# kurhula/pyABC

Measured on AMD Instinct MI355X. Metric: accepted particles/sec/generation, higher is better.
Workload: dtype f32 (f16x3-limb MFMA, f32-grade)

## Files before the change

### include/abcgpu.h

```cpp
#ifndef ABCGPU_H
#define ABCGPU_H

#include <stddef.h>
#include <stdint.h>

#ifdef __cplusplus
extern "C" {
#endif

#define ABC_OK 0
#define ABC_ERR_INVALID (-1)
#define ABC_ERR_HIP (-2)
#define ABC_ERR_WORKSPACE (-3)
#define ABC_ERR_NOT_ENOUGH_PARTICLES (-4)
#define ABC_ERR_UNSUPPORTED (-5)
#define ABC_ERR_COMM (-6)

#define ABC_MAX_D 2048

#define ABC_PREC_F64 0
#define ABC_PREC_F32 1
#define ABC_PREC_X3 2

#define ABC_PRIOR_FLAT (-1)
#define ABC_PRIOR_NORM 0
#define ABC_PRIOR_UNIFORM 1
#define ABC_PRIOR_EXPON 2
#define ABC_PRIOR_LAPLACE 3
#define ABC_PRIOR_LOGNORM 4
#define ABC_PRIOR_GAMMA 5
#define ABC_PRIOR_BETA 6
#define ABC_PRIOR_HOST 7

const char* abc_last_error(void);
int abc_version(void);

int abc_profile_begin(void);
int abc_profile_end(double* total_ms, int64_t* launches);
#define ABC_PROF_DENSITY 0
#define ABC_PROF_CANDIDATES 1
#define ABC_PROF_REGEN 2
#define ABC_PROF_RESCUE 3
int abc_profile_channel(int channel, double* total_ms, int64_t* launches);

size_t abc_weighted_moments_workspace(int64_t N, int d);
int abc_weighted_moments(const double* X, const double* w, int64_t N, int d,
                         double* out, void* ws, size_t ws_bytes, void* stream);

size_t abc_scan_workspace(int64_t N);
int abc_inclusive_scan_f64(const double* in, double* out, int64_t N, void* ws,
                           size_t ws_bytes, void* stream);

size_t abc_normalize_weights_workspace(int64_t N);
int abc_normalize_weights(double* w, int64_t N, double* stats, void* ws,
                          size_t ws_bytes, void* stream);

size_t abc_mvn_packed_bytes(int64_t N, int r, int prec);
int abc_mvn_pack_population(const double* X, const double* w, int64_t N, int d,
                            const double* mu, const double* U, int r,
                            double log_w_shift, const double* log_w_shift_dev,
                            int prec, void* packed, double* range, void* stream);
int abc_mvn_fit(const double* moments, int d, double scaling, int bw_rule,
                double* cov, double* evec, double* evals, double* U, double* L,
                double* stats, void* stream);
size_t abc_mvn_logpdf_workspace(int64_t M, int64_t N, int r, int prec);
int abc_mvn_x3_layout(int r, int* kslots, int* tiles_per_wave);
int abc_mvn_x3_max_exponent(void);
int abc_mvn_logpdf(const double* x, int64_t M, int d, const void* packed,
                   const double* X, const double* w, int64_t N,
                   const double* mu, const double* U, int r, int prec,
                   double log_const, double log_w_shift, double* out,
                   const int64_t* hint_rows, void* ws, size_t ws_bytes,
                   void* stream);
int abc_mvn_logpdf_direct(const double* x, int64_t M, const double* X,
                          const double* w, int64_t N, int d, const double* U,
                          int r, const double* V, int nv, double support_tol,
                          double log_const, double* out, void* stream);

int abc_cdf_guide(const double* cdf, int64_t N, int32_t* guide, void* stream);
int abc_propose(const double* X, const double* cdf, const int32_t* guide,
                int64_t N, int d, const double* L, const int32_t* prior_kind,
                const double* prior_params, uint64_t seed, uint32_t generation,
                int64_t idx0, int64_t B, int max_attempts, double* theta,
                double* prior_logpdf, int64_t* ancestor, int32_t* attempts,
                void* stream);
int abc_prior_logpdf(const double* theta, int64_t B, int d,
                     const int32_t* prior_kind, const double* prior_params,
                     double* out, void* stream);
int abc_prior_uniforms(const int32_t* attempts, double* u, int64_t B, int k,
                       uint64_t seed, uint32_t generation, int64_t idx0,
                       void* stream);

int abc_simulate_linear_gaussian(const double* theta, int64_t B, int d, int S,
                                 const int32_t* src, const double* a,
                                 const double* sigma, uint64_t seed,
                                 uint32_t generation, int64_t idx0, double* x,
                                 void* stream);

int abc_pnorm(const double* x, int64_t B, int S, const double* x0,
              const double* wf, double p, double* d, void* stream);

int abc_mask_gave_up(double* dist, const int32_t* attempts, int64_t B,
                     int max_attempts, double value, void* stream);

size_t abc_compact_workspace(int64_t B);
int abc_accept_compact(const double* d, int64_t B, double eps, int64_t* idx,
                       int64_t* count, void* ws, size_t ws_bytes,
                       void* stream);
typedef struct abc_candidate_spec {
  int d;
  int S;
  const double* X;
  const double* cdf;
  const int32_t* guide;
  int64_t N;
  const double* L;
  int per_particle_L;
  const int32_t* prior_kind;
  const double* prior_params;
  int max_attempts;
  const int32_t* src;
  const double* a;
  const double* sigma;
  const double* x0;
  const double* wf;
  double p;
  uint64_t seed;
  uint32_t generation;
  const void* anc_table;
  const double* support_box;
} abc_candidate_spec;
int abc_prior_support_box(const int32_t* prior_kind, const double* prior_params, int d,
                          double* box, void* stream);
int64_t abc_ancestor_table_bytes(int64_t N, int d);
int abc_ancestor_table(const double* X, const double* cdf, int64_t N, int d,
                       void* table, size_t table_bytes, void* stream);
size_t abc_candidates_workspace(int64_t B);
int abc_candidates_round(const abc_candidate_spec* spec, int64_t idx0,
                         int64_t B, double eps, const double* eps_dev,
                         double eps_scale, int filter, int64_t cap,
                         int64_t* idx, int64_t* count, double* rec_x,
                         void* ws, size_t ws_bytes, void* stream);
int abc_round_keep(const int64_t* counts, int nranks, int rank, int64_t need, int64_t* keep,
                   void* stream);
int abc_candidates_regen(const abc_candidate_spec* spec, int64_t idx0,
                         const int64_t* idx, int64_t n, const int64_t* n_dev,
                         double* theta, double* prior_logpdf, int64_t* ancestor,
                         double* x, double* dist, void* stream);

size_t abc_candidates_propose_workspace(void);
int abc_candidates_propose(const abc_candidate_spec* spec, int64_t idx0, int64_t B,
                           double* theta, double* prior_logpdf, int64_t* ancestor,
                           int32_t* attempts, void* ws, size_t ws_bytes, void* stream);

int abc_pnorm_accept(const double* x, int64_t B, int S, const double* x0,
                     const double* wf, double p, double eps, const int32_t* attempts,
                     int max_attempts, int64_t cap, int64_t* idx, int64_t* count,
                     void* ws, size_t ws_bytes, void* stream);

#define ABC_AGG_MAX_TERMS 16
int abc_aggregate_distance(const double* x, int64_t B, int S, const double* x0,
                           const double* wf, const double* p, const double* c, int K,
                           double* d, double* terms, void* stream);
int abc_aggregate_accept(const double* x, int64_t B, int S, const double* x0,
                         const double* wf, const double* p, const double* c, int K,
                         double eps, const int32_t* attempts, int max_attempts, int64_t cap,
                         int64_t* idx, int64_t* count, void* ws, size_t ws_bytes,
                         void* stream);

int abc_gather_rows(const double* in, const int64_t* idx, int64_t n, int cols,
                    double* out, void* stream);
int abc_gather_rows_batch(int n_arrays, const double* const* ins,
                          const int* cols, double* const* outs,
                          const int64_t* out_row0, const int64_t* idx,
                          int64_t n, void* stream);

int abc_importance_weights(const double* prior_logpdf,
                           const double* trans_logpdf,
                           const double* acc_weights, int64_t A, double scale,
                           double* w, void* stream);

size_t abc_sort_pairs_workspace(int64_t N);
int abc_sort_pairs_f64(const double* keys, const double* vals, int64_t N,
                       double* keys_out, double* vals_out, void* ws,
                       size_t ws_bytes, void* stream);
size_t abc_weighted_quantile_workspace(int64_t N);
int abc_weighted_quantile(const double* points, const double* w, int64_t N,
                          double alpha, double* q, void* ws, size_t ws_bytes,
                          void* stream);
size_t abc_weighted_quantile_sorted_workspace(int64_t N);
int abc_weighted_quantile_sorted(const double* points, const double* w, int64_t N,
                                 double alpha, double* q, void* ws, size_t ws_bytes,
                                 void* stream);

size_t abc_column_stats_workspace(int64_t R, int S);
int abc_column_std(const double* X, int64_t R, int S, double* out, void* ws,
                   size_t ws_bytes, void* stream);
int abc_column_mad(const double* X, int64_t R, int S, double* out, void* ws,
                   size_t ws_bytes, void* stream);

enum { ABC_SCALE_MAD, ABC_SCALE_MEAN_AD, ABC_SCALE_STD, ABC_SCALE_BIAS, ABC_SCALE_RMSD,
       ABC_SCALE_MAD_TO_OBS, ABC_SCALE_MEAN_AD_TO_OBS, ABC_SCALE_CMAD,
       ABC_SCALE_CMEAN_AD, ABC_SCALE_STD_TO_OBS };
size_t abc_column_scale_workspace(int kind, int64_t R, int S);
int abc_column_scale(int kind, const double* X, int64_t R, int S, const double* x0,
                     double* out, void* ws, size_t ws_bytes, void* stream);

int abc_column_span(const double* V, int64_t R, int K, double* out, void* ws,
                    size_t ws_bytes, void* stream);

size_t abc_local_fit_workspace(int64_t N, int d);
int abc_local_fit(const double* X, const double* w, int64_t N, int d,
                  int64_t k, double scaling, double eps, double* covs,
                  double* inv_covs, double* dets, double* chol,
                  double* log_norm, void* ws, size_t ws_bytes, void* stream);
#define ABC_FIT_KNN 1
#define ABC_FIT_LIST 2
#define ABC_FIT_DENSE 4
#define ABC_FIT_DEFER 8
#define ABC_FIT_DENSE_REJECTED 16
#define ABC_FIT_SELECT_FALLBACK 32
int abc_local_fit_route(void);
size_t abc_local_logpdf_workspace(int64_t M, int64_t N, int d);
int abc_local_logpdf(const double* x, int64_t M, const double* X,
                     const double* w, int64_t N, int d, const double* inv_covs,
                     const double* log_norm, double* out, void* ws,
                     size_t ws_bytes, void* stream);
int abc_local_logpdf_route(int64_t M, int64_t N, int d, void* ws, size_t ws_bytes,
                           void* stream, int64_t* direct, double* bound);
int abc_local_propose(const double* X, const double* cdf,
                      const int32_t* guide, int64_t N, int d,
                      const double* chol, const int32_t* prior_kind,
                      const double* prior_params, uint64_t seed,
                      uint32_t generation, int64_t idx0, int64_t B,
                      int max_attempts, double* theta, double* prior_logpdf,
                      int64_t* ancestor, int32_t* attempts, void* stream);

size_t abc_bootstrap_cv_workspace(int64_t N);
int abc_bootstrap_cv(const double* logdens, int64_t B, int64_t N,
                     const double* w, double scale, double* variation,
                     double* cv, void* ws, size_t ws_bytes, void* stream);

int abc_kernel_logpdf(const double* x, int64_t B, int S, const int32_t* cols,
                      int K, const double* x0k, int kind, const double* par,
                      const double* U, int r, double c, int ret_lin,
                      double* out, void* stream);
int abc_stochastic_accept(const double* dens, int64_t B, double pdf_norm,
                          double temperature, int scale_log, int apply_iw,
                          uint64_t seed, uint32_t generation, int64_t idx0,
                          double* key, double* accw, void* stream);
size_t abc_temper_workspace(void);
int abc_temper_sums(const double* dens, const double* lr,
                    const double* lr_sub, int64_t R, double pdf_norm, int scale_log, int mode, double beta,
                    double shift, double* out, void* ws, size_t ws_bytes,
                    void* stream);

#define ABC_COMM_ID_BYTES 128
#define ABC_COMM_F64 0
#define ABC_COMM_I64 1
#define ABC_COMM_SUM 0
#define ABC_COMM_MAX 1
#define ABC_COMM_MIN 2
int abc_comm_unique_id(void* id);
int abc_comm_init(void** comm, int nranks, int rank, const void* id);
int abc_comm_destroy(void* comm);
int abc_comm_allgather(void* comm, const void* send, void* recv, size_t bytes,
                       void* stream);
int abc_comm_allreduce(void* comm, const void* send, void* recv, size_t count,
                       int dtype, int op, void* stream);
int abc_comm_broadcast(void* comm, void* buf, size_t bytes, int root, void* stream);

#ifdef __cplusplus
}
#endif
#endif
```

### pyabc_amd/_native.py

```python
import ctypes as C
import os
import threading

_HERE = os.path.dirname(os.path.abspath(__file__))
LIB_PATH = os.environ.get("ABCGPU_LIB", os.path.join(_HERE, "libabcgpu.so"))

P = C.c_void_p
I64 = C.c_int64
I32 = C.c_int
D = C.c_double
U64 = C.c_uint64
U32 = C.c_uint32
SZ = C.c_size_t

SIGNATURES = {
    "abc_last_error": (C.c_char_p, []),
    "abc_version": (I32, []),
    "abc_profile_begin": (I32, []),
    "abc_profile_end": (I32, [P, P]),
    "abc_profile_channel": (I32, [I32, P, P]),
    "abc_weighted_moments_workspace": (SZ, [I64, I32]),
    "abc_weighted_moments": (I32, [P, P, I64, I32, P, P, SZ, P]),
    "abc_scan_workspace": (SZ, [I64]),
    "abc_inclusive_scan_f64": (I32, [P, P, I64, P, SZ, P]),
    "abc_normalize_weights_workspace": (SZ, [I64]),
    "abc_normalize_weights": (I32, [P, I64, P, P, SZ, P]),
    "abc_mvn_packed_bytes": (SZ, [I64, I32, I32]),
    "abc_mvn_x3_layout": (I32, [I32, P, P]),
    "abc_mvn_x3_max_exponent": (I32, []),
    "abc_mvn_pack_population": (I32, [P, P, I64, I32, P, P, I32, D, P, I32, P, P,
                                      P]),
    "abc_mvn_fit": (I32, [P, I32, D, I32, P, P, P, P, P, P, P]),
    "abc_mvn_logpdf_workspace": (SZ, [I64, I64, I32, I32]),
    "abc_mvn_logpdf": (I32, [P, I64, I32, P, P, P, I64, P, P, I32, I32, D, D,
                             P, P, P, SZ, P]),
    "abc_mvn_logpdf_direct": (I32, [P, I64, P, P, I64, I32, P, I32, P, I32,
                                    D, D, P, P]),
    "abc_cdf_guide": (I32, [P, I64, P, P]),
    "abc_ancestor_table_bytes": (I64, [I64, I32]),
    "abc_ancestor_table": (I32, [P, P, I64, I32, P, SZ, P]),
    "abc_propose": (I32, [P, P, P, I64, I32, P, P, P, U64, U32, I64, I64, I32,
                          P, P, P, P, P]),
    "abc_prior_logpdf": (I32, [P, I64, I32, P, P, P, P]),
    "abc_prior_uniforms": (I32, [P, P, I64, I32, U64, U32, I64, P]),
    "abc_simulate_linear_gaussian": (I32, [P, I64, I32, I32, P, P, P, U64,
                                           U32, I64, P, P]),
    "abc_pnorm": (I32, [P, I64, I32, P, P, D, P, P]),
    "abc_mask_gave_up": (I32, [P, P, I64, I32, D, P]),
    "abc_compact_workspace": (SZ, [I64]),
    "abc_accept_compact": (I32, [P, I64, D, P, P, P, SZ, P]),
    "abc_candidates_workspace": (SZ, [I64]),
    "abc_prior_support_box": (I32, [P, P, I32, P, P]),
    "abc_round_keep": (I32, [P, I32, I32, I64, P, P]),
    "abc_candidates_round": (I32, [P, I64, I64, D, P, D, I32, I64, P, P, P, P, SZ, P]),
    "abc_candidates_regen": (I32, [P, I64, P, I64, P, P, P, P, P, P, P]),
    "abc_pnorm_accept": (I32, [P, I64, I32, P, P, D, D, P, I32, I64, P, P, P, SZ, P]),
    "abc_aggregate_distance": (I32, [P, I64, I32, P, P, P, P, I32, P, P, P]),
    "abc_aggregate_accept": (I32, [P, I64, I32, P, P, P, P, I32, D, P, I32, I64, P, P, P,
                                   SZ, P]),
    "abc_column_span": (I32, [P, I64, I32, P, P, SZ, P]),
    "abc_candidates_propose_workspace": (SZ, []),
    "abc_candidates_propose": (I32, [P, I64, I64, P, P, P, P, P, SZ, P]),
    "abc_gather_rows": (I32, [P, P, I64, I32, P, P]),
    "abc_gather_rows_batch": (I32, [I32, P, P, P, P, P, I64, P]),
    "abc_importance_weights": (I32, [P, P, P, I64, D, P, P]),
    "abc_sort_pairs_workspace": (SZ, [I64]),
    "abc_sort_pairs_f64": (I32, [P, P, I64, P, P, P, SZ, P]),
    "abc_weighted_quantile_workspace": (SZ, [I64]),
    "abc_weighted_quantile": (I32, [P, P, I64, D, P, P, SZ, P]),
    "abc_weighted_quantile_sorted_workspace": (SZ, [I64]),
    "abc_weighted_quantile_sorted": (I32, [P, P, I64, D, P, P, SZ, P]),
    "abc_column_stats_workspace": (SZ, [I64, I32]),
    "abc_column_std": (I32, [P, I64, I32, P, P, SZ, P]),
    "abc_column_mad": (I32, [P, I64, I32, P, P, SZ, P]),
    "abc_column_scale_workspace": (SZ, [I32, I64, I32]),
    "abc_column_scale": (I32, [I32, P, I64, I32, P, P, P, SZ, P]),
    "abc_local_fit_workspace": (SZ, [I64, I32]),
    "abc_local_fit": (I32, [P, P, I64, I32, I64, D, D, P, P, P, P, P, P, SZ,
                            P]),
    "abc_local_fit_route": (I32, []),
    "abc_local_logpdf_workspace": (SZ, [I64, I64, I32]),
    "abc_local_logpdf": (I32, [P, I64, P, P, I64, I32, P, P, P, P, SZ, P]),
    "abc_local_logpdf_route": (I32, [I64, I64, I32, P, SZ, P, P, P]),
    "abc_local_propose": (I32, [P, P, P, I64, I32, P, P, P, U64, U32, I64,
                                I64, I32, P, P, P, P, P]),
    "abc_bootstrap_cv_workspace": (SZ, [I64]),
    "abc_bootstrap_cv": (I32, [P, I64, I64, P, D, P, P, P, SZ, P]),
    "abc_kernel_logpdf": (I32, [P, I64, I32, P, I32, P, I32, P, P, I32, D,
                                I32, P, P]),
    "abc_stochastic_accept": (I32, [P, I64, D, D, I32, I32, U64, U32, I64,
                                    P, P, P]),
    "abc_temper_workspace": (SZ, []),
    "abc_temper_sums": (I32, [P, P, P, I64, D, I32, I32, D, D, P, P, SZ, P]),
    "abc_comm_unique_id": (I32, [P]),
    "abc_comm_init": (I32, [P, I32, I32, P]),
    "abc_comm_destroy": (I32, [P]),
    "abc_comm_allgather": (I32, [P, P, P, SZ, P]),
    "abc_comm_allreduce": (I32, [P, P, P, SZ, I32, I32, P]),
    "abc_comm_broadcast": (I32, [P, P, SZ, I32, P]),
}



class CandidateSpec(C.Structure):
    _fields_ = [("d", C.c_int), ("S", C.c_int),
                ("X", P), ("cdf", P), ("guide", P), ("N", I64),
                ("L", P), ("per_particle_L", C.c_int),
                ("prior_kind", P), ("prior_params", P), ("max_attempts", C.c_int),
                ("src", P), ("a", P), ("sigma", P),
                ("x0", P), ("wf", P), ("p", D),
                ("seed", U64), ("generation", U32), ("anc_table", P),
                ("support_box", P)]


ABC_OK = 0
ABC_ERR_INVALID = -1
ABC_ERR_HIP = -2
ABC_ERR_WORKSPACE = -3
ABC_ERR_NOT_ENOUGH_PARTICLES = -4
ABC_ERR_UNSUPPORTED = -5
ABC_ERR_COMM = -6
ABC_AGG_MAX_TERMS = 16
ABC_COMM_ID_BYTES = 128
ABC_COMM_F64, ABC_COMM_I64 = 0, 1
ABC_COMM_SUM, ABC_COMM_MAX, ABC_COMM_MIN = 0, 1, 2
ABC_PROF_DENSITY, ABC_PROF_CANDIDATES, ABC_PROF_REGEN, ABC_PROF_RESCUE = 0, 1, 2, 3
(ABC_FIT_KNN, ABC_FIT_LIST, ABC_FIT_DENSE, ABC_FIT_DEFER, ABC_FIT_DENSE_REJECTED,
 ABC_FIT_SELECT_FALLBACK) = 1, 2, 4, 8, 16, 32
ABC_PREC_F64 = 0
ABC_PREC_F32 = 1
ABC_PREC_X3 = 2
(ABC_SCALE_MAD, ABC_SCALE_MEAN_AD, ABC_SCALE_STD, ABC_SCALE_BIAS, ABC_SCALE_RMSD,
 ABC_SCALE_MAD_TO_OBS, ABC_SCALE_MEAN_AD_TO_OBS, ABC_SCALE_CMAD, ABC_SCALE_CMEAN_AD,
 ABC_SCALE_STD_TO_OBS) = range(10)
SCALE_KINDS = {"mad": ABC_SCALE_MAD, "mean_ad": ABC_SCALE_MEAN_AD,
               "std": ABC_SCALE_STD, "bias": ABC_SCALE_BIAS,
               "rmsd": ABC_SCALE_RMSD, "mad_to_obs": ABC_SCALE_MAD_TO_OBS,
               "mean_ad_to_obs": ABC_SCALE_MEAN_AD_TO_OBS,
               "cmad": ABC_SCALE_CMAD, "cmean_ad": ABC_SCALE_CMEAN_AD,
               "std_to_obs": ABC_SCALE_STD_TO_OBS}

PRIOR_KINDS = {"norm": 0, "uniform": 1, "expon": 2, "laplace": 3,
               "lognorm": 4, "gamma": 5, "beta": 6, "host": 7}


class NativeError(RuntimeError):
    def __init__(self, fn, code, msg):
        super().__init__(f"{fn} failed ({code}): {msg}")
        self.code = code


_lib = None
_lock = threading.Lock()


def load():
    global _lib
    if _lib is not None:
        return _lib
    with _lock:
        if _lib is not None:
            return _lib
        if not os.path.exists(LIB_PATH):
            raise ImportError(
                f"libabcgpu.so not found at {LIB_PATH}; build it with "
                "`python -m pyabc_amd.build` (hipcc, gfx950)")
        lib = C.CDLL(LIB_PATH)
        for name, (res, args) in SIGNATURES.items():
            fn = getattr(lib, name)
            fn.restype = res
            fn.argtypes = args
        _lib = lib
    return _lib


def call(name, *args):
    lib = load()
    rc = getattr(lib, name)(*args)
    if rc != ABC_OK:
        msg = lib.abc_last_error().decode(errors="replace")
        if rc == ABC_ERR_INVALID:
            raise ValueError(f"{name}: {msg}")
        raise NativeError(name, rc, msg)
    return rc


def query(name, *args):
    return int(getattr(load(), name)(*args))
```

### pyabc_amd/csrc/abc_candidate.h

```cpp
#pragma once
#include "abc_common.h"

#pragma clang fp contract(off)

namespace abc {

constexpr double LOG_SQRT_2PI = 0.91893853320467274178;
constexpr uint32_t SLOTS_PER_ATTEMPT = 65536;
constexpr uint32_t SLOT_ANCESTOR = 0;
constexpr uint32_t SLOT_PERTURB = 1;
constexpr uint32_t SLOT_PRIOR = 32;
constexpr uint32_t SLOT_SIM = 0x40000000u;

__device__ __forceinline__ void normals4(uint64_t g, uint32_t slot, uint32_t gen,
                                         uint64_t seed, double n[4], int need = 4,
                                         const float* tab = BM_TAB) {
  u32x4 r = philox(g, slot, gen, seed);
  box_muller(r.x, r.y, n[0], n[1], tab);
  if (need > 2) box_muller(r.z, r.w, n[2], n[3], tab);
}

__device__ __forceinline__ void perturb_words(int p, const u32x4& anc, u32x4& r, uint64_t g,
                                              uint32_t s0, uint32_t gen, uint64_t seed,
                                              uint32_t& wa, uint32_t& wb) {
  if (p == 0) {
    wa = anc.z;
    wb = anc.w;
    return;
  }
  const int p1 = p - 1;
  if ((p1 & 1) == 0) r = philox(g, s0 + SLOT_PERTURB + (uint32_t)(p1 >> 1), gen, seed);
  wa = (p1 & 1) ? r.z : r.x;
  wb = (p1 & 1) ? r.w : r.y;
}

__device__ __noinline__ double prior_logpdf1(int kind, const double* p, double x) {
  switch (kind) {
    case ABC_PRIOR_FLAT:
      return 0.0;
    case ABC_PRIOR_NORM: {
      double y = (x - p[0]) / p[1];
      return -0.5 * (y * y) - LOG_SQRT_2PI - log(p[1]);
    }
    case ABC_PRIOR_UNIFORM: {
      double y = (x - p[0]) / p[1];
      return (y >= 0.0 && y <= 1.0) ? -log(p[1]) : -INFINITY;
    }
    case ABC_PRIOR_EXPON: {
      double y = (x - p[0]) / p[1];
      return (y >= 0.0) ? -y - log(p[1]) : -INFINITY;
    }
    case ABC_PRIOR_LAPLACE: {
      double y = (x - p[0]) / p[1];
      return -fabs(y) - log(2.0 * p[1]);
    }
    case ABC_PRIOR_LOGNORM: {
      double y = (x - p[1]) / p[2];
      if (!(y > 0.0)) return -INFINITY;
      const double lg = log(y), ly = lg / p[0];
      return -0.5 * ly * ly - lg - log(p[0]) - LOG_SQRT_2PI - log(p[2]);
    }
    case ABC_PRIOR_GAMMA: {
      double a = p[0], y = (x - p[1]) / p[2];
      if (y < 0.0) return -INFINITY;
      if (y == 0.0) return a < 1.0 ? INFINITY : (a == 1.0 ? -log(p[2]) : -INFINITY);
      const double t1 = (a == 1.0) ? 0.0 : (a - 1.0) * log(y);
      return t1 - y - lgamma(a) - log(p[2]);
    }
    case ABC_PRIOR_BETA: {
      double a = p[0], b = p[1], y = (x - p[2]) / p[3];
      if (y < 0.0 || y > 1.0) return -INFINITY;
      double lb = lgamma(a) + lgamma(b) - lgamma(a + b);
      double t1 = (a == 1.0) ? 0.0 : (a - 1.0) * log(y);
      double t2 = (b == 1.0) ? 0.0 : (b - 1.0) * log1p(-y);
      return t1 + t2 - lb - log(p[3]);
    }
    case ABC_PRIOR_HOST:
      return (x >= p[0] && x <= p[1]) ? 0.0 : -INFINITY;
  }
  return NAN;
}

__device__ __forceinline__ bool prior_in_support1(int kind, const double* p, double x) {
  switch (kind) {
    case ABC_PRIOR_FLAT:
      return true;
    case ABC_PRIOR_NORM: {
      double y = (x - p[0]) / p[1];
      return y * y < INFINITY;
    }
    case ABC_PRIOR_UNIFORM: {
      double y = (x - p[0]) / p[1];
      return y >= 0.0 && y <= 1.0;
    }
    case ABC_PRIOR_EXPON: {
      double y = (x - p[0]) / p[1];
      return y >= 0.0 && y < INFINITY;
    }
    case ABC_PRIOR_LAPLACE: {
      double y = (x - p[0]) / p[1];
      return fabs(y) < INFINITY;
    }
    case ABC_PRIOR_LOGNORM: {
      double y = (x - p[1]) / p[2];
      return y > 0.0 && y < INFINITY;
    }
    case ABC_PRIOR_GAMMA: {
      double y = (x - p[1]) / p[2];
      return (y > 0.0 && y < INFINITY) || (y == 0.0 && p[0] <= 1.0);
    }
    case ABC_PRIOR_BETA: {
      double y = (x - p[2]) / p[3];
      if (!(y >= 0.0 && y <= 1.0)) return false;
      if (y == 0.0 && p[0] > 1.0) return false;
      if (y == 1.0 && p[1] > 1.0) return false;
      return true;
    }
    case ABC_PRIOR_HOST:
      return x >= p[0] && x <= p[1];
  }
  return false;
}

__device__ inline double gamma_draw(double a, uint64_t g, uint32_t base, uint32_t gen,
                                    uint64_t seed) {
  double boost = 1.0;
  uint32_t it = 0;
  if (a < 1.0) {
    u32x4 r = philox(g, base + 500, gen, seed);
    boost = pow(uniform01(r.x), 1.0 / a);
    a += 1.0;
  }
  const double dd = a - 1.0 / 3.0, c = 1.0 / sqrt(9.0 * dd);
  for (; it < 480; ++it) {
    u32x4 r = philox(g, base + it, gen, seed);
    double n0, n1;
    box_muller(r.x, r.y, n0, n1);
    double v = 1.0 + c * n0;
    if (v <= 0.0) continue;
    v = v * v * v;
    double u = uniform01(r.z);
    if (log(u) < 0.5 * n0 * n0 + dd - dd * v + dd * log(v)) return dd * v * boost;
  }
  return dd * boost;
}

__device__ __noinline__ double prior_draw1(int kind, const double* p, uint64_t g,
                                     uint32_t base, uint32_t gen, uint64_t seed) {
  u32x4 r = philox(g, base, gen, seed);
  double n0, n1;
  switch (kind) {
    case ABC_PRIOR_NORM:
      box_muller(r.x, r.y, n0, n1);
      return p[0] + p[1] * n0;
    case ABC_PRIOR_UNIFORM:
      return p[0] + p[1] * uniform53(r.x, r.y);
    case ABC_PRIOR_EXPON:
      return p[0] - p[1] * log(uniform01(r.x));
    case ABC_PRIOR_LAPLACE: {
      double u = uniform01(r.x) - 0.5;
      return p[0] - p[1] * copysign(1.0, u) * log1p(-2.0 * fabs(u));
    }
    case ABC_PRIOR_LOGNORM:
      box_muller(r.x, r.y, n0, n1);
      return p[1] + p[2] * exp(p[0] * n0);
    case ABC_PRIOR_GAMMA:
      return p[1] + p[2] * gamma_draw(p[0], g, base + 1, gen, seed);
    case ABC_PRIOR_BETA: {
      double x = gamma_draw(p[0], g, base + 1, gen, seed);
      double y = gamma_draw(p[1], g, base + 1 + 256, gen, seed);
      return p[2] + p[3] * x / (x + y);
    }
    case ABC_PRIOR_HOST:
      return p[2];
  }
  return NAN;
}

__device__ __forceinline__ double prior_logpdf(const int32_t* kind,
                                               const double* params, int d,
                                               const double* th) {
  double s = 0.0;
  for (int k = 0; k < d; ++k) s += prior_logpdf1(kind[k], params + 4 * k, th[k]);
  return s;
}

__device__ __forceinline__ int64_t upper_bound(const double* cdf, int64_t N,
                                               double target) {
  int64_t lo = 0, hi = N;
  while (lo < hi) {
    int64_t mid = (lo + hi) >> 1;
    if (cdf[mid] > target) hi = mid; else lo = mid + 1;
  }
  return lo < N ? lo : N - 1;
}

__device__ __forceinline__ int64_t ancestor_search(const double* __restrict__ cdf,
                                                   const int32_t* __restrict__ guide,
                                                   int64_t N, double total,
                                                   double target) {
  if (guide == nullptr) return upper_bound(cdf, N, target);
  const double step = total / (double)N;
  int64_t k = (int64_t)floor(target / step) - 1;
  k = k < 0 ? 0 : (k > N - 1 ? N - 1 : k);
  int64_t lo = guide[k];
  int64_t hi = k + 3 < N ? (int64_t)guide[k + 3] + 1 : N;
  while (lo < hi) {
    const int64_t mid = (lo + hi) >> 1;
    if (cdf[mid] > target) hi = mid; else lo = mid + 1;
  }
  return lo < N ? lo : N - 1;
}

struct AncestorBracket { int64_t lo, hi; };
__device__ __forceinline__ AncestorBracket ancestor_bracket(const int32_t* __restrict__ guide,
                                                            int64_t N, double total,
                                                            double target) {
  if (guide == nullptr) return {0, N};
  const double step = total / (double)N;
  int64_t k = (int64_t)floor(target / step) - 1;
  k = k < 0 ? 0 : (k > N - 1 ? N - 1 : k);
  const int64_t k3 = k + 3 < N ? k + 3 : N - 1;
  const int64_t lo = guide[k];
  const int64_t g3 = guide[k3];
  return {lo, k + 3 < N ? g3 + 1 : N};
}
__device__ __forceinline__ int64_t ancestor_finish(const double* __restrict__ cdf, int64_t N,
                                                   double target, AncestorBracket b) {
  int64_t lo = b.lo, hi = b.hi;
  while (lo < hi) {
    const int64_t mid = (lo + hi) >> 1;
    if (cdf[mid] > target) hi = mid; else lo = mid + 1;
  }
  return lo < N ? lo : N - 1;
}

__device__ __forceinline__ int64_t table_finish(const double* __restrict__ rec, int rs, int d,
                                                int64_t N, double target, AncestorBracket b) {
  int64_t lo = b.lo, hi = b.hi;
  while (lo < hi) {
    const int64_t mid = (lo + hi) >> 1;
    if (rec[mid * rs + d] > target) hi = mid; else lo = mid + 1;
  }
  return lo < N ? lo : N - 1;
}

__device__ __forceinline__ uint64_t dkey(double x) {
  const uint64_t u = (uint64_t)__double_as_longlong(x);
  return (u >> 63) ? ~u : (u | (1ull << 63));
}
__device__ __forceinline__ double dval(uint64_t k) {
  const uint64_t u = (k >> 63) ? (k & ~(1ull << 63)) : ~k;
  return __longlong_as_double((long long)u);
}
__device__ __forceinline__ void support_bounds_wave(int kind, const double* pg, double* lo_hi) {
  const int lane = threadIdx.x & 63;
  double p[4];
#pragma unroll
  for (int i = 0; i < 4; ++i) p[i] = pg[i];
  double c;
  switch (kind) {
    case ABC_PRIOR_UNIFORM: c = p[0] + 0.5 * p[1]; break;
    case ABC_PRIOR_EXPON: c = p[0] + p[1]; break;
    case ABC_PRIOR_LOGNORM: case ABC_PRIOR_GAMMA: c = p[1] + p[2]; break;
    case ABC_PRIOR_BETA: c = p[2] + 0.5 * p[3]; break;
    case ABC_PRIOR_NORM: case ABC_PRIOR_LAPLACE: c = p[0]; break;
    case ABC_PRIOR_HOST: c = p[2]; break;
    default: c = 0.0;
  }
  auto pos = [](double v) { return v > 0.0 && v < INFINITY; };
  bool dom = true;
  switch (kind) {
    case ABC_PRIOR_NORM: case ABC_PRIOR_UNIFORM: case ABC_PRIOR_EXPON: case ABC_PRIOR_LAPLACE:
      dom = pos(p[1]); break;
    case ABC_PRIOR_LOGNORM: case ABC_PRIOR_GAMMA: dom = pos(p[0]) && pos(p[2]); break;
    case ABC_PRIOR_BETA: dom = pos(p[0]) && pos(p[1]) && pos(p[3]); break;
    default: break;
  }
  if (!dom || !prior_in_support1(kind, p, c)) {
    bool found = false;
    if (dom && fabs(c) < INFINITY) {
      const uint64_t kc0 = dkey(c);
#pragma unroll
      for (int s = 0; s < 2; ++s) {
        double c2 = dval(s ? kc0 - 1 : kc0 + 1);
        if (c2 == c) c2 = dval(s ? kc0 - 2 : kc0 + 2);
        if (!found && prior_in_support1(kind, p, c2)) {
          c = c2;
          found = true;
        }
      }
    }
    if (!found) {
      if (lane == 0) { lo_hi[0] = INFINITY; lo_hi[1] = -INFINITY; }
      return;
    }
  }
  auto turn = [&](uint64_t lo, uint64_t hi, bool up) {
    while (hi - lo > 1) {
      const uint64_t span = hi - lo;
      const uint64_t step = span / 65 > 0 ? span / 65 : 1;
      const uint64_t m = lo + step * (uint64_t)(lane + 1);
      const bool inside = m < hi;
      const bool pr = inside ? (prior_in_support1(kind, p, dval(m)) == up) : true;
      const unsigned long long bal = __ballot(pr);
      if (bal == 0ull) {
        lo = lo + step * 64ull;
        continue;
      }
      const int f = __ffsll((long long)bal) - 1;
      const uint64_t mf = lo + step * (uint64_t)(f + 1);
      const uint64_t new_hi = mf < hi ? mf : hi;
      const uint64_t new_lo = f == 0 ? lo : lo + step * (uint64_t)f;
      lo = new_lo;
      hi = new_hi;
    }
    return hi;
  };
  const uint64_t kc = dkey(c);
  uint64_t lo_key;
  if (prior_in_support1(kind, p, -INFINITY)) lo_key = dkey(-INFINITY);
  else lo_key = turn(dkey(-INFINITY), kc, true);
  uint64_t hi_key;
  if (prior_in_support1(kind, p, INFINITY)) hi_key = dkey(INFINITY);
  else hi_key = turn(kc, dkey(INFINITY), false) - 1;
  if (lane == 0) { lo_hi[0] = dval(lo_key); lo_hi[1] = dval(hi_key); }
}

struct ProposalArgs {
  const double* X;
  const double* cdf;
  const int32_t* guide;
  int64_t N;
  const double* L;
  const int32_t* kind;
  const double* params;
  int d;
  int max_attempts;
  uint64_t seed;
  uint32_t gen;
  const double* rec = nullptr;
  const int32_t* bguide = nullptr;
  int rs = 0;
  int64_t G = 0;
  const double* xmax = nullptr;
};

constexpr int ANC_HDR = 256;
__host__ __device__ inline int anc_rs(int d) { return (d + 1 + 15) / 16 * 16; }
__host__ __device__ inline int64_t anc_bins(int64_t N) {
  const int64_t g = 4 * N;
  return g < (int64_t)0x7FFFFFF0 ? g : (int64_t)0x7FFFFFF0;
}
__device__ __forceinline__ int64_t anc_bin(double x, double inv_step, int64_t G) {
  const double b = x * inv_step;
  return b >= (double)G ? G : (int64_t)b;
}

constexpr int PROP_MVN = 0, PROP_LOCAL = 1, PROP_PRIOR = 2;
using PropModes = std::integer_sequence<int, PROP_MVN, PROP_LOCAL, PROP_PRIOR>;
inline int proposal_mode(const double* X, bool per_particle_L) {
  return X == nullptr ? PROP_PRIOR : (per_particle_L ? PROP_LOCAL : PROP_MVN);
}

using CandDims = std::integer_sequence<int, 1, 2, 3, 4, 5, 6, 8, 10, 12, 16>;

template <class F>
void dispatch_candidate(int d, int mode, F&& f) {
  auto with_d = [&](auto D) { dispatch_int(PropModes{}, mode, [&](auto MODE) { f(D, MODE); }); };
  if (!dispatch_int(CandDims{}, d, with_d)) with_d(std::integral_constant<int, 0>{});
}

struct SimDistArgs {
  const int32_t* src;
  const double* a;
  const double* sigma;
  const double* x0;
  const double* wf;
  double p;
  int S;
};

constexpr int SIM_SMAX = 256;
constexpr int LT_DMAX = 16;
struct BlockConsts {
  float bmt[BM_TAB_SIZE];
  double LT[LT_DMAX * LT_DMAX];
  double box[2 * 64];
  double2 as[SIM_SMAX];
  double2 wx[SIM_SMAX];
  int32_t src[SIM_SMAX];
  double total;
  double inv_step;
  int lazy;
};

template <int D, int MODE, bool BOX_FROM_SRC = false>
__device__ __forceinline__ void stage_block_consts(BlockConsts& C, const ProposalArgs& A,
                                                   const SimDistArgs* M,
                                                   const double* box_src) {
  const int t = threadIdx.x, nt = blockDim.x;
  const int d = D > 0 ? D : A.d;
  for (int k = t; k < BM_TAB_SIZE; k += nt) C.bmt[k] = BM_TAB[k];
  if (MODE == PROP_MVN && D > 0 && D <= LT_DMAX)
    for (int e = t; e < d * d; e += nt) C.LT[(e % d) * d + e / d] = A.L[e];
  if (BOX_FROM_SRC) {
    for (int k = t; k < 2 * d; k += nt) C.box[k] = box_src[k];
  } else {
    for (int k = t >> 6; k < d; k += nt >> 6)
      support_bounds_wave(A.kind[k], A.params + 4 * k, C.box + 2 * k);
  }
  if (M)
    for (int k = t; k < M->S && k < SIM_SMAX; k += nt) {
      C.as[k] = make_double2(M->a[k], M->sigma[k]);
      C.wx[k] = make_double2(M->wf[k], M->x0[k]);
      C.src[k] = M->src[k];
    }
  if (t == 0) {
    const double total = (MODE != PROP_PRIOR) ? A.cdf[A.N - 1] : 0.0;
    C.total = total;
    C.inv_step = (MODE != PROP_PRIOR && A.rec) ? (double)A.G / total : 0.0;
  }
  __syncthreads();
}

template <int D, int MODE, bool TABLE = false>
__device__ __forceinline__ int propose_one(const ProposalArgs& A, const BlockConsts& C,
                                           uint64_t g, double* th, int64_t& j) {
  constexpr bool LT_LDS = MODE == PROP_MVN && D > 0 && D <= LT_DMAX;
  const int d = D > 0 ? D : A.d;
  j = -1;
  const double total = C.total;
  for (int att = 0; att < A.max_attempts; ++att) {
    const uint32_t s0 = (uint32_t)att * SLOTS_PER_ATTEMPT;
    int oz = 0;
    asm volatile("" : "+s"(oz));
    const double* LT = C.LT + oz;
    const double* box = C.box + oz;
    if (MODE == PROP_PRIOR) {
#pragma unroll
      for (int k = 0; k < (D > 0 ? D : d); ++k)
        th[k] = prior_draw1(A.kind[k], A.params + 4 * k, g,
                            s0 + SLOT_PRIOR + 512u * k, A.gen, A.seed);
    } else {
      const u32x4 ra = philox(g, s0 + SLOT_ANCESTOR, A.gen, A.seed);
      u32x4 r = ra;
      const double target = uniform53(ra.x, ra.y) * total;
      AncestorBracket br;
      if (TABLE) {
        const int64_t kt = anc_bin(target, C.inv_step, A.G);
        br = {A.bguide[kt], A.bguide[kt + 1]};
      } else {
        br = ancestor_bracket(A.guide, A.N, total, target);
      }
#pragma unroll
      for (int k = 0; k < (D > 0 ? D : d); ++k) th[k] = 0.0;
      const double* Lj = A.L;
      if (MODE == PROP_LOCAL) {
        j = TABLE ? table_finish(A.rec, A.rs, d, A.N, target, br)
                  : ancestor_finish(A.cdf, A.N, target, br);
        Lj = A.L + j * d * d;
      }
      auto pair = [&](int q) {
        uint32_t wa, wb;
        perturb_words(q >> 1, ra, r, g, s0, A.gen, A.seed, wa, wb);
        double n0, n1;
        box_muller(wa, wb, n0, n1, C.bmt);
        const bool two = q + 1 < d;
#pragma unroll
        for (int k = 0; k < (D > 0 ? D : d); ++k) {
          if (k >= q) {
            const double l0 = LT_LDS ? LT[q * d + k] : Lj[k * d + q];
            th[k] = fma(l0, n0, th[k]);
          }
          if (two && k >= q + 1) {
            const double l1 = LT_LDS ? LT[(q + 1) * d + k] : Lj[k * d + q + 1];
            th[k] = fma(l1, n1, th[k]);
          }
        }
      };
#pragma unroll 1
      for (int q = 0; q < d; q += 2) pair(q);
      if (MODE != PROP_LOCAL)
        j = TABLE ? table_finish(A.rec, A.rs, d, A.N, target, br)
                  : ancestor_finish(A.cdf, A.N, target, br);
      const double* Xj = TABLE ? A.rec + j * A.rs : A.X + j * d;
#pragma unroll
      for (int k = 0; k < (D > 0 ? D : d); ++k) th[k] = Xj[k] + th[k];
    }
    bool ok = true;
#pragma unroll
    for (int k = 0; k < (D > 0 ? D : d); ++k)
      ok = ok & (box[2 * k] <= th[k]) & (th[k] <= box[2 * k + 1]);
    if (ok) return att + 1;
  }
  return A.max_attempts + 1;
}

constexpr int LAZY_KT = 4;

template <int D, int MODE>
__device__ __forceinline__ bool lazy_filter_ok(const BlockConsts& C, const ProposalArgs& A,
                                               const SimDistArgs& M) {
  if constexpr (MODE != PROP_MVN || D <= LAZY_KT || D > LT_DMAX) {
    return false;
  } else {
    if (A.xmax == nullptr || M.S <= 4) return false;
    bool ok = true;
    for (int k = 0; k < 4; ++k) ok = ok && C.src[k] >= 0 && C.src[k] < LAZY_KT;
    const double xm = *A.xmax;
    for (int k = LAZY_KT; k < D; ++k) {
      double ls = 0.0;
      for (int q = 0; q <= k; ++q) ls += fabs(C.LT[q * D + k]);
      const double b = (xm + 7.6 * ls) * 1.000001 + 1e-300;
      ok = ok && (C.box[2 * k] <= -b) && (b <= C.box[2 * k + 1]);
    }
    return ok;
  }
}

__device__ __forceinline__ double pterm(double v, double p) {
#pragma clang fp contract(off)
  return (p == 1.0) ? v : (p == 2.0 ? v * v : pow(v, p));
}
template <int PK = 0>
__device__ __forceinline__ double pnorm_acc(double s, double v, double p) {
#pragma clang fp contract(off)
  if constexpr (PK == 2) return s + v * v;
  return isinf(p) ? fmax(s, v) : s + pterm(v, p);
}
template <int PK = 0>
__device__ __forceinline__ double pnorm_finish(double s, double p) {
#pragma clang fp contract(off)
  if constexpr (PK == 2) return sqrt(s);
  return isinf(p) ? s : ((p == 1.0) ? s : (p == 2.0 ? sqrt(s) : pow(s, 1.0 / p)));
}
__device__ __forceinline__ double pnorm_row(const double* xr, int S, const double* x0,
                                            const double* wf, double p) {
#pragma clang fp contract(off)
  double s = 0.0;
  if (isinf(p)) {
    for (int k = 0; k < S; ++k) s = fmax(s, fabs(wf[k] * (xr[k] - x0[k])));
    return pnorm_finish<0>(s, p);
  }
  for (int k = 0; k < S; ++k) s += pterm(fabs(wf[k] * (xr[k] - x0[k])), p);
  return pnorm_finish<0>(s, p);
}
constexpr int PNORM_ROWS = 8;
template <class F>
__device__ __forceinline__ void pnorm_wave_rows(const double* x, int64_t b0, int64_t B, int S,
                                                const double* x0, const double* wf, double p,
                                                F&& emit) {
#pragma clang fp contract(off)
  const int lane = threadIdx.x & 63;
  const bool inf = isinf(p);
  double s[PNORM_ROWS];
#pragma unroll
  for (int r = 0; r < PNORM_ROWS; ++r) s[r] = 0.0;
  for (int k = lane; k < S; k += 64) {
    const double wk = wf[k], ck = x0[k];
    double v[PNORM_ROWS];
#pragma unroll
    for (int r = 0; r < PNORM_ROWS; ++r) v[r] = b0 + r < B ? x[(b0 + r) * S + k] : ck;
#pragma unroll
    for (int r = 0; r < PNORM_ROWS; ++r) {
      const double a = fabs(wk * (v[r] - ck));
      s[r] = inf ? fmax(s[r], a) : s[r] + pterm(a, p);
    }
  }
#pragma unroll
  for (int r = 0; r < PNORM_ROWS; ++r) {
    const double t = inf ? wave_max(s[r]) : wave_sum(s[r]);
    if (lane == 0 && b0 + r < B) emit(r, pnorm_finish<0>(t, p));
  }
}

__device__ __forceinline__ double lg_stat(double a, double sigma, double th_src, double e) {
  return a * th_src + sigma * e;
}

template <int PK = 0>
__device__ __forceinline__ double sim_pnorm_range(const SimDistArgs& M, const BlockConsts& C,
                                                  const double* tsrc, int tstride,
                                                  uint64_t g, uint32_t gen,
                                                  uint64_t seed, int q0, int q1,
                                                  double s, double* x, int xoff = 0) {
  u32x4 r;
  if (q0 < q1 && (q0 & 3)) r = philox(g, SLOT_SIM + (uint32_t)(q0 >> 2), gen, seed);
#pragma unroll 1
  for (int q = q0; q < q1; q += 2) {
    if ((q & 3) == 0) r = philox(g, SLOT_SIM + (uint32_t)(q >> 2), gen, seed);
    double n2[2];
    box_muller((q & 2) ? r.z : r.x, (q & 2) ? r.w : r.y, n2[0], n2[1], C.bmt);
#pragma unroll
    for (int t = 0; t < 2; ++t) {
      const int k = q + t;
      if (k < q1) {
        const double2 as = C.as[k], wx = C.wx[k];
        const double xv = lg_stat(as.x, as.y, tsrc[C.src[k] * tstride], n2[t]);
        if (x) x[k - xoff] = xv;
        s = pnorm_acc<PK>(s, fabs(wx.x * (xv - wx.y)), M.p);
      }
    }
  }
  return s;
}

template <int D, int PK = 0>
__device__ __forceinline__ double sim_pnorm_regs(const SimDistArgs& M, const BlockConsts& C,
                                                 const double (&th)[D], uint64_t g,
                                                 uint32_t gen, uint64_t seed, int q0, int q1,
                                                 double s, double* x, int xoff = 0) {
  u32x4 r;
  if (q0 < q1 && (q0 & 3)) r = philox(g, SLOT_SIM + (uint32_t)(q0 >> 2), gen, seed);
#pragma unroll 1
  for (int q = q0; q < q1; q += 2) {
    if ((q & 3) == 0) r = philox(g, SLOT_SIM + (uint32_t)(q >> 2), gen, seed);
    double n2[2];
    box_muller((q & 2) ? r.z : r.x, (q & 2) ? r.w : r.y, n2[0], n2[1], C.bmt);
#pragma unroll
    for (int t = 0; t < 2; ++t) {
      const int k = q + t;
      if (k < q1) {
        const double2 as = C.as[k], wx = C.wx[k];
        const int sk = __builtin_amdgcn_readfirstlane(C.src[k]);
        const double xv = lg_stat(as.x, as.y, th[sk], n2[t]);
        if (x) x[k - xoff] = xv;
        s = pnorm_acc<PK>(s, fabs(wx.x * (xv - wx.y)), M.p);
      }
    }
  }
  return s;
}

template <int D, int PK = 0>
__device__ __forceinline__ double sim_pnorm(const SimDistArgs& M, const BlockConsts& C,
                                            const double* th, uint64_t g, uint32_t gen,
                                            uint64_t seed, int q0, int q1, double s, double* x,
                                            int xoff = 0) {
  if constexpr (D > 0) {
    return sim_pnorm_regs<D, PK>(M, C, *reinterpret_cast<const double(*)[D]>(th), g, gen, seed,
                                 q0, q1, s, x, xoff);
  } else {
    return sim_pnorm_range<PK>(M, C, th, 1, g, gen, seed, q0, q1, s, x, xoff);
  }
}

template <int D, int PK, int CG>
__device__ __forceinline__ void lazy_head_group(const ProposalArgs& A, const SimDistArgs& M,
                                                const BlockConsts& C, const uint64_t (&g)[CG],
                                                double eps, bool (&keep)[CG]) {
  constexpr int KT = LAZY_KT;
  static_assert(D > KT, "lazy_head_group: D > LAZY_KT");
  int oz = 0;
  asm volatile("" : "+s"(oz));
  const double* LT = C.LT + oz;
  const double* box = C.box + oz;
  double target[CG];
  int32_t glo[CG], ghi[CG];
  uint32_t az[CG], aw[CG];
#pragma unroll
  for (int c = 0; c < CG; ++c) {
    const u32x4 r = philox(g[c], SLOT_ANCESTOR, A.gen, A.seed);
    target[c] = uniform53(r.x, r.y) * C.total;
    az[c] = r.z;
    aw[c] = r.w;
    const int64_t kt = anc_bin(target[c], C.inv_step, A.G);
    glo[c] = A.bguide[kt];
    ghi[c] = A.bguide[kt + 1];
  }
  double th[CG][KT];
#pragma unroll
  for (int c = 0; c < CG; ++c) {
#pragma unroll
    for (int k = 0; k < KT; ++k) th[c][k] = 0.0;
    const u32x4 r = philox(g[c], SLOT_PERTURB, A.gen, A.seed);
#pragma unroll
    for (int q = 0; q < KT; q += 2) {
      double n0, n1;
      box_muller(q == 0 ? az[c] : r.x, q == 0 ? aw[c] : r.y, n0, n1, C.bmt);
#pragma unroll
      for (int k = 0; k < KT; ++k) {
        if (k >= q) th[c][k] = fma(LT[q * D + k], n0, th[c][k]);
        if (k >= q + 1) th[c][k] = fma(LT[(q + 1) * D + k], n1, th[c][k]);
      }
    }
  }
  const double* xh[CG];
#pragma unroll
  for (int c = 0; c < CG; ++c) {
    const int64_t j = table_finish(A.rec, A.rs, D, A.N, target[c],
                                   AncestorBracket{(int64_t)glo[c], (int64_t)ghi[c]});
    xh[c] = A.rec + j * A.rs;
  }
  double xv4[CG][KT];
#pragma unroll
  for (int c = 0; c < CG; ++c)
#pragma unroll
    for (int k = 0; k < KT; ++k) xv4[c][k] = xh[c][k];
  double e[CG][4];
#pragma unroll
  for (int c = 0; c < CG; ++c) {
    const u32x4 r = philox(g[c], SLOT_SIM, A.gen, A.seed);
    box_muller(r.x, r.y, e[c][0], e[c][1], C.bmt);
    box_muller(r.z, r.w, e[c][2], e[c][3], C.bmt);
  }
#pragma unroll
  for (int c = 0; c < CG; ++c) {
    bool ok = true;
#pragma unroll
    for (int k = 0; k < KT; ++k) {
      th[c][k] = xv4[c][k] + th[c][k];
      ok = ok & (box[2 * k] <= th[c][k]) & (th[c][k] <= box[2 * k + 1]);
    }
    double s = 0.0;
#pragma unroll
    for (int k = 0; k < 4; ++k) {
      const double2 as = C.as[k], wx = C.wx[k];
      const int sk = __builtin_amdgcn_readfirstlane(C.src[k]);
      const double xv = lg_stat(as.x, as.y, th[c][sk], e[c][k]);
      s = pnorm_acc<PK>(s, fabs(wx.x * (xv - wx.y)), M.p);
    }
    keep[c] = !ok || !(pnorm_finish<PK>(s, M.p) > eps);
  }
}

}
```

### pyabc_amd/csrc/abc_fused.hip

```cpp
#include "abc_candidate.h"
#include "abc_aggregate.h"

namespace abc {
namespace {

constexpr int FR_T = 256;
constexpr int FR_CPT = 8;
constexpr int FR_TILE = FR_T * FR_CPT;
constexpr int FR_WORDS = FR_TILE / 64;
constexpr int FR_CG = 2;

struct RoundArgs {
  ProposalArgs P;
  SimDistArgs M;
  const double* box;
  const double* eps_dev;
  double eps_scale;
};

template <int D, int MODE, int PK>
__device__ __forceinline__ double evaluate_full(const RoundArgs& A, const BlockConsts& C,
                                                uint64_t g,
                                                double* th, int64_t& j, int& att, double* x) {
  att = propose_one<D, MODE, true>(A.P, C, g, th, j);
  const double s = sim_pnorm<D, PK>(A.M, C, th, g, A.P.gen, A.P.seed, 0, A.M.S, 0.0, x);
  const double dist = pnorm_finish<PK>(s, A.M.p);
  return att <= A.P.max_attempts ? dist : NAN;
}

constexpr int XCH = 16;
template <int D, int MODE, int PK>
__device__ __forceinline__ double evaluate_staged(const RoundArgs& A, const BlockConsts& C,
                                                  uint64_t g, bool valid, double* th,
                                                  int64_t& j, int& att, double* out,
                                                  int nvalid, double (*stage)[XCH + 1]) {
  const int t = threadIdx.x;
  const int S = A.M.S;
  att = valid ? propose_one<D, MODE, true>(A.P, C, g, th, j) : A.P.max_attempts + 1;
  double s = 0.0;
  for (int k0 = 0; k0 < S; k0 += XCH) {
    const int k1 = k0 + XCH < S ? k0 + XCH : S;
    if (valid) s = sim_pnorm<D, PK>(A.M, C, th, g, A.P.gen, A.P.seed, k0, k1, s, stage[t], k0);
    __syncthreads();
    const int w = k1 - k0;
    for (int e = t; e < FR_T * w; e += FR_T) {
      const int r = e / w, c = e - r * w;
      if (r < nvalid) out[(int64_t)r * S + k0 + c] = stage[r][c];
    }
    __syncthreads();
  }
  const double dist = pnorm_finish<PK>(s, A.M.p);
  return att <= A.P.max_attempts ? dist : NAN;
}

__device__ __forceinline__ void flush_accept_words(const uint32_t* tbits, int nwords,
                                                   int64_t tile0, int64_t B, uint64_t* bits) {
  const int lane = threadIdx.x & 63, wave = threadIdx.x >> 6;
  if (wave == 0 && lane < nwords) {
    const uint64_t w = (uint64_t)tbits[2 * lane] | ((uint64_t)tbits[2 * lane + 1] << 32);
    const int64_t word = tile0 / 64 + lane;
    if (word * 64 < B) bits[word] = w;
  }
}

struct TileLds {
  uint32_t* tbits;
  uint16_t* queue;
  int& qn;
};
template <int D, int MODE, bool FILTER, int PK>
__device__ __forceinline__ void tile_body(const RoundArgs& A, const BlockConsts& C, double eps,
                                          int64_t idx0, int64_t B, int64_t tile0, int cpt,
                                          uint64_t* __restrict__ bits,
                                          double* __restrict__ rec_x, TileLds T) {
  constexpr int DM = D > 0 ? D : 64;
  const int tid = threadIdx.x;
  const int tn = cpt * FR_T;
  if (tid < tn / 32) T.tbits[tid] = 0u;
  if (tid == 0) T.qn = 0;
  __syncthreads();
  double th[DM];
  int64_t j;
  int att;
  if (FILTER) {
    bool lazy_done = false;
    if constexpr (MODE == PROP_MVN && D > LAZY_KT && D <= LT_DMAX) {
      if (C.lazy) {
#pragma unroll 1
        for (int it = 0; it < cpt; it += FR_CG) {
          uint64_t gs[FR_CG];
          bool keep[FR_CG];
#pragma unroll
          for (int c = 0; c < FR_CG; ++c) gs[c] = (uint64_t)(idx0 + tile0 + (it + c) * FR_T + tid);
          lazy_head_group<D, PK, FR_CG>(A.P, A.M, C, gs, eps, keep);
#pragma unroll
          for (int c = 0; c < FR_CG; ++c) {
            const int loc = (it + c) * FR_T + tid;
            if (keep[c] && tile0 + loc < B) {
              const int pos = atomicAdd(&T.qn, 1);
              T.queue[pos] = (uint16_t)loc;
            }
          }
        }
        lazy_done = true;
      }
    }
#pragma unroll 1
    for (int it = 0; it < (lazy_done ? 0 : cpt); ++it) {
      const int loc = it * FR_T + tid;
      const int64_t b = tile0 + loc;
      if (b < B) {
        const uint64_t g = (uint64_t)(idx0 + b);
        att = propose_one<D, MODE, true>(A.P, C, g, th, j);
        const double s = sim_pnorm<D, PK>(A.M, C, th, g, A.P.gen, A.P.seed, 0, 4, 0.0, nullptr);
        if (att <= A.P.max_attempts && !(pnorm_finish<PK>(s, A.M.p) > eps)) {
          const int pos = atomicAdd(&T.qn, 1);
          T.queue[pos] = (uint16_t)loc;
        }
      }
    }
    __syncthreads();
  }
  const int n = FILTER ? T.qn : tn;
#pragma unroll 1
  for (int i = tid; i < n; i += FR_T) {
    const int loc = FILTER ? (int)T.queue[i] : i;
    const int64_t b = tile0 + loc;
    if (b < B) {
      double* xr = rec_x ? rec_x + b * A.M.S : nullptr;
      const double dist = evaluate_full<D, MODE, PK>(A, C, (uint64_t)(idx0 + b), th, j, att,
                                                  xr);
      if (dist <= eps) atomicOr(&T.tbits[loc >> 5], 1u << (loc & 31));
    }
  }
  __syncthreads();
  flush_accept_words(T.tbits, tn / 64, tile0, B, bits);
}

constexpr int FR_CPT_TAIL = 2;
constexpr int FR_TILE_TAIL = FR_T * FR_CPT_TAIL;

struct TilePlan {
  int64_t nbig, ntiles;
  unsigned int grid;
};
__host__ __device__ inline void tile_span(int64_t t, int64_t nbig, int64_t& tile0, int& cpt) {
  if (t < nbig) { tile0 = t * FR_TILE; cpt = FR_CPT; }
  else { tile0 = nbig * FR_TILE + (t - nbig) * FR_TILE_TAIL; cpt = FR_CPT_TAIL; }
}

template <int D, int MODE, bool FILTER, int PK>
__device__ __forceinline__ void round_body(RoundArgs A, int64_t idx0, int64_t B,
                                           double eps_host, uint64_t* __restrict__ bits,
                                           unsigned int* __restrict__ ticket,
                                           int64_t nbig, int64_t ntiles,
                                           double* __restrict__ rec_x) {
  const double eps = A.eps_dev ? (*A.eps_dev) * A.eps_scale : eps_host;
  __shared__ BlockConsts C;
  __shared__ uint32_t tbits[FR_TILE / 32];
  __shared__ uint16_t queue[FR_TILE];
  __shared__ int qn;
  __shared__ int64_t s_tile;
  const TileLds T{tbits, queue, qn};
  stage_block_consts<D, MODE, true>(C, A.P, &A.M, A.box);
  if (FILTER) {
    if (threadIdx.x == 0) C.lazy = lazy_filter_ok<D, MODE>(C, A.P, A.M) ? 1 : 0;
  }
  const unsigned int limit = (unsigned int)(ntiles + gridDim.x - 1);
#pragma unroll 1
  for (;;) {
    if (threadIdx.x == 0) s_tile = (int64_t)atomicInc(ticket, limit);
    __syncthreads();
    const int64_t t = s_tile;
    if (t >= ntiles) break;
    int64_t tile0;
    int cpt;
    tile_span(t, nbig, tile0, cpt);
    tile_body<D, MODE, FILTER, PK>(A, C, eps, idx0, B, tile0, cpt, bits, rec_x, T);
    __syncthreads();
  }
}

template <int D, int MODE, int PK>
__device__ __forceinline__ void round_plain_body(RoundArgs A, int64_t idx0, int64_t B,
                                                 double eps_host, uint64_t* __restrict__ bits,
                                                 unsigned int* __restrict__ ticket,
                                                 int64_t nbig, int64_t ntiles,
                                                 double* __restrict__ rec_x) {
  const double eps = A.eps_dev ? (*A.eps_dev) * A.eps_scale : eps_host;
  constexpr int DM = D > 0 ? D : 64;
  __shared__ BlockConsts C;
  __shared__ uint32_t tbits[FR_TILE / 32];
  __shared__ int64_t s_tile;
  stage_block_consts<D, MODE, true>(C, A.P, &A.M, A.box);
  const int tid = threadIdx.x, lane = tid & 63, wave = tid >> 6;
  const unsigned int limit = (unsigned int)(ntiles + gridDim.x - 1);
  int64_t tile0 = 0;
  int cpt = 0, it = 0;
  bool started = false;
#pragma unroll 1
  for (;;) {
    if (it == cpt) {
      __syncthreads();
      if (started && wave == 0 && lane < cpt * (FR_T / 64)) {
        const uint64_t w = (uint64_t)tbits[2 * lane] | ((uint64_t)tbits[2 * lane + 1] << 32);
        const int64_t word = tile0 / 64 + lane;
        if (word * 64 < B) bits[word] = w;
      }
      if (tid == 0) s_tile = (int64_t)atomicInc(ticket, limit);
      __syncthreads();
      const int64_t t = (int64_t)(((uint64_t)(uint32_t)__builtin_amdgcn_readfirstlane(
                                       (int)(s_tile >> 32)) << 32) |
                                  (uint32_t)__builtin_amdgcn_readfirstlane((int)s_tile));
      if (t >= ntiles) break;
      tile_span(t, nbig, tile0, cpt);
      if (tid < FR_TILE / 32) tbits[tid] = 0u;
      __syncthreads();
      it = 0;
      started = true;
    }
    const int loc = it * FR_T + tid;
    const int64_t b = tile0 + loc;
    if (b < B) {
      double th[DM];
      int64_t j;
      int att;
      double* xr = rec_x ? rec_x + b * A.M.S : nullptr;
      const double dist = evaluate_full<D, MODE, PK>(A, C, (uint64_t)(idx0 + b), th, j, att, xr);
      if (dist <= eps) atomicOr(&tbits[loc >> 5], 1u << (loc & 31));
    }
    ++it;
  }
}

__host__ __device__ constexpr int fr_min_waves(bool filter, int D, int MODE, int PK) {
  return (!filter && PK == 2 && D == 10 && MODE != PROP_PRIOR) ? 6 : 1;
}

#define ABC_ROUND_KERNEL(NAME, FILTER, PK)                                                \
  template <int D, int MODE>                                                              \
  __global__ __launch_bounds__(FR_T, fr_min_waves(FILTER, D, MODE, PK))                   \
  void NAME(RoundArgs A, int64_t idx0, int64_t B,                                         \
                                               double eps, uint64_t* bits,                \
                                               unsigned int* ticket, int64_t nbig,        \
                                               int64_t ntiles, double* rec_x) {           \
    if (FILTER)                                                                           \
      round_body<D, MODE, true, PK>(A, idx0, B, eps, bits, ticket, nbig, ntiles, nullptr);\
    else                                                                                  \
      round_plain_body<D, MODE, PK>(A, idx0, B, eps, bits, ticket, nbig, ntiles, rec_x);  \
  }
ABC_ROUND_KERNEL(fused_round_plain, false, 0)
ABC_ROUND_KERNEL(fused_round_plain_p2, false, 2)
ABC_ROUND_KERNEL(fused_round_filter, true, 0)
ABC_ROUND_KERNEL(fused_round_filter_p2, true, 2)
#undef ABC_ROUND_KERNEL

constexpr int RG_MAX = 2048;
constexpr int RG_T = 256;

__global__ __launch_bounds__(RG_T) void bits_range_sum_kernel(
    const uint64_t* __restrict__ bits, int64_t nwords, int64_t wpr,
    int64_t* __restrict__ rtot) {
  __shared__ int ws[RG_T / 64];
  const int64_t w0 = (int64_t)blockIdx.x * wpr;
  const int64_t w1 = w0 + wpr < nwords ? w0 + wpr : nwords;
  int c = 0;
  for (int64_t w = w0 + threadIdx.x; w < w1; w += RG_T) c += __popcll(bits[w]);
#pragma unroll
  for (int o = 32; o > 0; o >>= 1) c += __shfl_xor(c, o, 64);
  if ((threadIdx.x & 63) == 0) ws[threadIdx.x >> 6] = c;
  __syncthreads();
  if (threadIdx.x == 0) {
    int64_t tot = 0;
    for (int q = 0; q < RG_T / 64; ++q) tot += ws[q];
    rtot[blockIdx.x] = tot;
  }
}

constexpr int WB = 32;
__global__ __launch_bounds__(256) void bits_write_ranges(
    const uint64_t* __restrict__ bits, int64_t nwords, int64_t wpr, int nranges,
    const int64_t* __restrict__ rtot, int64_t cap, int64_t* __restrict__ idx,
    int64_t* __restrict__ count) {
  const int lane = threadIdx.x & 63;
  const int r = blockIdx.x * 4 + (threadIdx.x >> 6);
  if (r >= nranges) return;
  int64_t off = 0;
  for (int q = lane; q < r; q += 64) off += rtot[q];
#pragma unroll
  for (int o = 32; o > 0; o >>= 1) off += __shfl_xor(off, o, 64);
  const int64_t mine = rtot[r];
  if (r == nranges - 1 && lane == 0) *count = off + mine;
  if (off >= cap || mine == 0) return;
  const int64_t w0 = (int64_t)r * wpr;
  const int64_t w1 = w0 + wpr < nwords ? w0 + wpr : nwords;
  for (int64_t b0 = w0; b0 < w1 && off < cap; b0 += 64 * WB) {
    uint64_t w[WB];
#pragma unroll
    for (int q = 0; q < WB; ++q) {
      const int64_t wd = b0 + 64 * q + lane;
      w[q] = wd < w1 ? bits[wd] : 0ull;
    }
#pragma unroll
    for (int q = 0; q < WB; ++q) {
      if (b0 + 64 * q >= w1 || off >= cap) break;
      const int c = __popcll(w[q]);
      int incl = c;
#pragma unroll
      for (int o = 1; o < 64; o <<= 1) {
        const int u = __shfl_up(incl, o, 64);
        if (lane >= o) incl += u;
      }
      int64_t pos = off + (incl - c);
      uint64_t m = w[q];
      const int64_t wd = b0 + 64 * q + lane;
      while (m != 0ull && pos < cap) {
        idx[pos++] = wd * 64 + (__ffsll((long long)m) - 1);
        m &= m - 1;
      }
      off += __shfl(incl, 63, 64);
    }
  }
}

__global__ __launch_bounds__(64) void support_box_kernel(const int32_t* __restrict__ kind,
                                                         const double* __restrict__ params,
                                                         int d, double* __restrict__ box) {
  const int k = blockIdx.x;
  if (k < d) support_bounds_wave(kind[k], params + 4 * k, box + 2 * k);
}

struct Ranges { int64_t nwords, wpr; int n; };
inline Ranges make_ranges(int64_t B, int64_t most, int64_t least) {
  Ranges r;
  r.nwords = ceil_div(B, 64);
  if (most > RG_MAX) most = RG_MAX;
  int64_t n = ceil_div(r.nwords, least);
  n = n < most ? n : most;
  n = n < 1 ? 1 : n;
  r.wpr = ceil_div(r.nwords, n);
  r.n = (int)ceil_div(r.nwords, r.wpr);
  return r;
}

inline TilePlan plan_tiles(int64_t B, int resident) {
  TilePlan p;
  const int64_t tail = 2 * (int64_t)resident * FR_TILE_TAIL;
  p.nbig = B > tail ? (B - tail) / FR_TILE : 0;
  p.ntiles = p.nbig + ceil_div(B - p.nbig * FR_TILE, FR_TILE_TAIL);
  p.grid = (unsigned int)(p.ntiles < resident ? p.ntiles : resident);
  return p;
}

template <int D, int MODE>
void launch_round(bool filt, bool p2, const RoundArgs& A, int64_t idx0, int64_t B, double eps,
                  uint64_t* bits, unsigned int* ticket, double* rec_x, hipStream_t s) {
  auto k = filt ? (p2 ? fused_round_filter_p2<D, MODE> : fused_round_filter<D, MODE>)
                : (p2 ? fused_round_plain_p2<D, MODE> : fused_round_plain<D, MODE>);
  const TilePlan p = plan_tiles(B, resident_blocks(k, FR_T));
  hipLaunchKernelGGL(k, dim3(p.grid), dim3(FR_T), 0, s, A, idx0, B, eps, bits, ticket, p.nbig,
                     p.ntiles, rec_x);
}

template <int D, int MODE>
__global__ __launch_bounds__(256) void fused_regen_kernel(
    RoundArgs A, int64_t idx0, const int64_t* __restrict__ idx, int64_t n,
    const int64_t* __restrict__ n_dev, double* __restrict__ theta, double* __restrict__ lp,
    int64_t* __restrict__ anc, double* __restrict__ x, double* __restrict__ dist) {
  constexpr int DM = D > 0 ? D : 64;
  __shared__ BlockConsts C;
  __shared__ double stage[FR_T][XCH + 1];
  if (n_dev && *n_dev < n) n = *n_dev > 0 ? *n_dev : 0;
  if ((int64_t)blockIdx.x * FR_T >= n) return;
  stage_block_consts<D, MODE>(C, A.P, &A.M, nullptr);
  const int d = D > 0 ? D : A.P.d;
  const int64_t i0 = (int64_t)blockIdx.x * FR_T;
  const int64_t i = i0 + threadIdx.x;
  const bool valid = i < n;
  const int nvalid = n - i0 < FR_T ? (int)(n - i0) : FR_T;
  double th[DM];
  int64_t j = -1;
  int att;
  const double dd = evaluate_staged<D, MODE, 0>(A, C, valid ? (uint64_t)(idx0 + idx[i]) : 0ull,
                                                valid, th, j, att, x + i0 * A.M.S, nvalid, stage);
  if (!valid) return;
#pragma unroll
  for (int k = 0; k < (D > 0 ? D : d); ++k) theta[i * d + k] = th[k];
  lp[i] = att <= A.P.max_attempts ? prior_logpdf(A.P.kind, A.P.params, d, th) : -INFINITY;
  if (anc) anc[i] = j;
  dist[i] = dd;
}

__global__ void round_keep_kernel(const int64_t* __restrict__ counts, int rank, int64_t need,
                                  int64_t* __restrict__ keep) {
  if (threadIdx.x != 0) return;
  int64_t left = need > 0 ? need : 0, k = 0;
  for (int q = 0; q <= rank; ++q) {
    const int64_t c = counts[q] > 0 ? counts[q] : 0;
    const int64_t take = c < left ? c : left;
    if (q == rank) k = take;
    left -= take;
  }
  *keep = k;
}

constexpr int FP_CPT = 4;
template <int D, int MODE>
__global__ __launch_bounds__(256) void fused_propose_kernel(
    RoundArgs A, int64_t idx0, int64_t B, double* __restrict__ theta,
    double* __restrict__ lp, int64_t* __restrict__ anc, int32_t* __restrict__ att_out) {
  constexpr int DM = D > 0 ? D : 64;
  __shared__ BlockConsts C;
  stage_block_consts<D, MODE, true>(C, A.P, nullptr, A.box);
  const int d = D > 0 ? D : A.P.d;
  for (int c = 0; c < FP_CPT; ++c) {
    const int64_t i = ((int64_t)blockIdx.x * FP_CPT + c) * FR_T + threadIdx.x;
    if (i >= B) break;
    double th[DM];
    int64_t j = -1;
    const int att = propose_one<D, MODE, true>(A.P, C, (uint64_t)(idx0 + i), th, j);
    double* row = theta + i * d;
#pragma unroll
    for (int k = 0; k < DM; ++k)
      if (k < d) row[k] = th[k];
    if (lp) lp[i] = att <= A.P.max_attempts ? prior_logpdf(A.P.kind, A.P.params, d, th) : -INFINITY;
    if (anc) anc[i] = j;
    if (att_out) att_out[i] = att;
  }
}

__host__ __device__ constexpr int pa_chunk_rows(int S) {
  return (65536 / ((S + 1) * 8)) >= FR_T ? FR_T : ((65536 / ((S + 1) * 8)) & ~1);
}
template <bool WIDE>
__global__ __launch_bounds__(FR_T) void pnorm_accept_kernel(
    const double* __restrict__ x, int64_t B, int S, const double* __restrict__ x0,
    const double* __restrict__ wf, double p, double eps, const int32_t* __restrict__ att,
    int max_attempts, uint64_t* __restrict__ bits) {
  __shared__ uint32_t tbits[FR_TILE / 32];
  const int tid = threadIdx.x;
  const int64_t tile0 = (int64_t)blockIdx.x * FR_TILE;
  if (tid < FR_TILE / 32) tbits[tid] = 0u;
  __syncthreads();
  auto ok = [&](int64_t b) { return att == nullptr || att[b] <= max_attempts; };
  if (!WIDE) {
    extern __shared__ double pa_rows[];
    const int S1 = S + 1;
    const int RC = pa_chunk_rows(S);
    const int n16 = RC * S / 2;
    const int per = (n16 + FR_T - 1) / FR_T;
    double2 hold[16];
    auto fetch = [&](int it) {
      const int64_t e0 = (tile0 + (int64_t)it * RC) * S;
      const int64_t eend = B * S;
#pragma unroll
      for (int q = 0; q < 16; ++q) {
        if (q >= per) break;
        const int piece = q * FR_T + tid;
        const int64_t e = e0 + 2 * (int64_t)piece;
        if (piece < n16 && e + 1 < eend) {
          hold[q] = *reinterpret_cast<const double2*>(x + e);
        } else if (piece < n16 && e < eend) {
          hold[q] = double2{x[e], 0.0};
        }
      }
    };
    auto stash = [&]() {
#pragma unroll
      for (int q = 0; q < 16; ++q) {
        if (q >= per) break;
        const int piece = q * FR_T + tid;
        if (piece < n16) {
          const int e = 2 * piece;
          const int r0 = e / S, k0 = e - r0 * S;
          pa_rows[r0 * S1 + k0] = hold[q].x;
          const int r1 = (e + 1) / S, k1 = e + 1 - r1 * S;
          pa_rows[r1 * S1 + k1] = hold[q].y;
        }
      }
    };
    const int64_t rows = B - tile0 < FR_TILE ? B - tile0 : FR_TILE;
    const int nchunk = (int)((rows + RC - 1) / RC);
    fetch(0);
#pragma unroll 1
    for (int it = 0; it < nchunk; ++it) {
      __syncthreads();
      stash();
      __syncthreads();
      if (it + 1 < nchunk) fetch(it + 1);
      const int loc = it * RC + tid;
      const int64_t b = tile0 + loc;
      if (tid < RC && loc < FR_TILE && b < B) {
        const double dist = pnorm_row(pa_rows + tid * S1, S, x0, wf, p);
        if (dist <= eps && ok(b)) atomicOr(&tbits[loc >> 5], 1u << (loc & 31));
      }
    }
  } else {
#pragma unroll 1
    for (int r0 = (tid >> 6) * PNORM_ROWS; r0 < FR_TILE; r0 += 4 * PNORM_ROWS) {
      const int64_t b0 = tile0 + r0;
      if (b0 >= B) break;
      pnorm_wave_rows(x, b0, B, S, x0, wf, p, [&](int r, double dist) {
        const int loc = r0 + r;
        if (dist <= eps && ok(b0 + r)) atomicOr(&tbits[loc >> 5], 1u << (loc & 31));
      });
    }
  }
  __syncthreads();
  flush_accept_words(tbits, FR_WORDS, tile0, B, bits);
}

constexpr int AGG_TILE_ROW = FR_T, AGG_TILE_WAVE = 64;
template <bool WIDE, bool SIMPLE>
__global__ __launch_bounds__(FR_T) void aggregate_accept_kernel(
    const double* __restrict__ x, int64_t B, int S, const double* __restrict__ x0,
    const double* __restrict__ wf, const AggTerms T, double eps,
    const int32_t* __restrict__ att, int max_attempts, uint64_t* __restrict__ bits) {
  constexpr int TILE = WIDE ? AGG_TILE_WAVE : AGG_TILE_ROW;
  __shared__ uint32_t tbits[TILE / 32];
  const int tid = threadIdx.x;
  const int64_t tile0 = (int64_t)blockIdx.x * TILE;
  if (tid < TILE / 32) tbits[tid] = 0u;
  __syncthreads();
  auto ok = [&](int64_t b) { return att == nullptr || att[b] <= max_attempts; };
  if (!WIDE) {
    const int64_t b = tile0 + tid;
    if (b < B) {
      const double dist = agg_row(x + b * S, S, x0, wf, T, [](int, double) {});
      if (dist <= eps && ok(b)) atomicOr(&tbits[tid >> 5], 1u << (tid & 31));
    }
  } else {
#pragma unroll 1
    for (int r0 = (tid >> 6) * PNORM_ROWS; r0 < TILE; r0 += 4 * PNORM_ROWS) {
      const int64_t b0 = tile0 + r0;
      if (b0 >= B) break;
      agg_wave_rows<SIMPLE>(x, b0, B, S, x0, wf, T, [](int, int, double) {},
                            [&](int r, double dist) {
        const int loc = r0 + r;
        if (dist <= eps && ok(b0 + r)) atomicOr(&tbits[loc >> 5], 1u << (loc & 31));
      });
    }
  }
  __syncthreads();
  flush_accept_words(tbits, TILE / 64, tile0, B, bits);
}

int write_ranges(const uint64_t* bits, const Ranges& rg, const int64_t* rtot, int64_t cap,
                 int64_t* idx, int64_t* count, hipStream_t s) {
  hipLaunchKernelGGL(bits_write_ranges, dim3((unsigned)ceil_div(rg.n, 4)), dim3(256), 0, s,
                     bits, rg.nwords, rg.wpr, rg.n, rtot, cap, idx, count);
  ABC_LAUNCHED();
  return ABC_OK;
}

int compact_accept_bits(const uint64_t* bits, int64_t* rtot, int64_t B, int64_t cap,
                        int64_t* idx, int64_t* count, hipStream_t s) {
  const Ranges rg = make_ranges(B, RG_MAX, RG_T);
  hipLaunchKernelGGL(bits_range_sum_kernel, dim3((unsigned)rg.n), dim3(RG_T), 0, s, bits,
                     rg.nwords, rg.wpr, rtot);
  ABC_LAUNCHED();
  return write_ranges(bits, rg, rtot, cap, idx, count, s);
}

__global__ __launch_bounds__(256) void anc_records_kernel(const double* __restrict__ X,
                                                          const double* __restrict__ cdf,
                                                          int64_t N, int d, int rs,
                                                          double* __restrict__ rec) {
  const int64_t e = (int64_t)blockIdx.x * 256 + threadIdx.x;
  if (e >= N * rs) return;
  const int64_t i = e / rs;
  const int k = (int)(e - i * rs);
  rec[e] = k < d ? X[i * d + k] : (k == d ? cdf[i] : 0.0);
}

constexpr int XMAX_BLOCKS = 512;
__global__ __launch_bounds__(256) void anc_xmax_kernel(const double* __restrict__ X,
                                                       int64_t n,
                                                       unsigned long long* __restrict__ xmax_bits) {
  __shared__ unsigned long long wm[4];
  unsigned long long a = 0ull;
  for (int64_t e = (int64_t)blockIdx.x * 256 + threadIdx.x; e < n; e += (int64_t)gridDim.x * 256) {
    const unsigned long long b = (unsigned long long)__double_as_longlong(fabs(X[e]));
    a = b > a ? b : a;
  }
#pragma unroll
  for (int o = 32; o > 0; o >>= 1) {
    const unsigned long long b = __shfl_xor(a, o, 64);
    a = b > a ? b : a;
  }
  if ((threadIdx.x & 63) == 0) wm[threadIdx.x >> 6] = a;
  __syncthreads();
  if (threadIdx.x == 0) {
    unsigned long long m = 0ull;
    for (int w = 0; w < 4; ++w) m = wm[w] > m ? wm[w] : m;
    atomicMax(xmax_bits, m);
  }
}

__global__ __launch_bounds__(256) void anc_guide_kernel(const double* __restrict__ cdf,
                                                        int64_t N, int64_t G,
                                                        int32_t* __restrict__ guide) {
  const int64_t k = (int64_t)blockIdx.x * 256 + threadIdx.x;
  if (k > G + 1) return;
  const double inv_step = (double)G / cdf[N - 1];
  int64_t lo = 0, hi = N;
  while (lo < hi) {
    const int64_t mid = (lo + hi) >> 1;
    if (anc_bin(cdf[mid], inv_step, G) >= k) hi = mid; else lo = mid + 1;
  }
  guide[k] = (int32_t)lo;
}

struct AncTable { const double* rec; const int32_t* guide; int rs; int64_t G; const double* xmax; };
inline AncTable anc_table_view(const void* t, int64_t N, int d) {
  AncTable v;
  v.xmax = static_cast<const double*>(t);
  v.rs = anc_rs(d);
  v.G = anc_bins(N);
  v.rec = reinterpret_cast<const double*>(static_cast<const char*>(t) + ANC_HDR);
  v.guide = reinterpret_cast<const int32_t*>(v.rec + N * v.rs);
  return v;
}

RoundArgs round_args(const abc_candidate_spec* s, const double* box) {
  RoundArgs A;
  A.box = box;
  A.eps_dev = nullptr;
  A.eps_scale = 1.0;
  A.P = ProposalArgs{s->X, s->cdf, s->guide, s->N, s->L, s->prior_kind,
                     s->prior_params, s->d, s->max_attempts, s->seed, s->generation};
  if (s->X && s->anc_table) {
    const AncTable v = anc_table_view(s->anc_table, s->N, s->d);
    A.P.rec = v.rec;
    A.P.bguide = v.guide;
    A.P.rs = v.rs;
    A.P.G = v.G;
    A.P.xmax = v.xmax;
  }
  A.M = SimDistArgs{s->src, s->a, s->sigma, s->x0, s->wf, s->p, s->S};
  return A;
}

int check_spec(const abc_candidate_spec* s) {
  ABC_CHECK_ARG(s != nullptr, "candidates: null spec");
  ABC_CHECK_ARG(s->d >= 1 && s->d <= 64 && s->S >= 1, "candidates: bad d/S");
  if (s->S > SIM_SMAX)
    return set_error(ABC_ERR_UNSUPPORTED, "candidates: S > %d (use the staged kernels)",
                     SIM_SMAX);
  ABC_CHECK_ARG(s->max_attempts >= 1 && s->max_attempts < (1 << 15),
                "candidates: bad max_attempts");
  ABC_CHECK_ARG(s->prior_kind && s->prior_params && s->src && s->a && s->sigma && s->x0 &&
                s->wf, "candidates: null pointer");
  ABC_CHECK_ARG(s->X == nullptr || (s->cdf && s->L && s->N >= 1),
                "candidates: population needs cdf, L, N");
  ABC_CHECK_ARG(s->p >= 1.0, "candidates: p < 1");
  ABC_CHECK_ARG(s->X == nullptr || s->anc_table, "candidates: population needs anc_table");
  return ABC_OK;
}

template <class F>
void dispatch_spec(const abc_candidate_spec* spec, F&& f) {
  dispatch_candidate(spec->d, proposal_mode(spec->X, spec->per_particle_L != 0), f);
}

}
}

using namespace abc;

struct RoundWs {
  unsigned int* ticket; int64_t* rtot; double* box; uint64_t* bits;
  void carve(Carver& c, int64_t B) {
    ticket = c.take<unsigned int>(64);
    rtot = c.take<int64_t>(RG_MAX);
    box = c.take<double>(128);
    bits = c.take<uint64_t>((size_t)ceil_div(B > 0 ? B : 1, FR_TILE) * FR_WORDS);
  }
};

extern "C" size_t abc_candidates_workspace(int64_t B) { return measure<RoundWs>(B); }

extern "C" int64_t abc_ancestor_table_bytes(int64_t N, int d) {
  if (N < 1 || d < 1) return 0;
  return ANC_HDR + N * anc_rs(d) * (int64_t)sizeof(double) +
         (anc_bins(N) + 2) * (int64_t)sizeof(int32_t);
}

extern "C" int abc_ancestor_table(const double* X, const double* cdf, int64_t N, int d,
                                  void* table, size_t table_bytes, void* stream) {
  ABC_CHECK_ARG(N >= 1 && N < (1ll << 31) && d >= 1 && d <= 64,
                "ancestor_table: bad N/d");
  ABC_CHECK_ARG(X && cdf && table, "ancestor_table: null pointer");
  ABC_CHECK_ARG(((uintptr_t)table & 127) == 0, "ancestor_table: table not 128-B aligned");
  if ((int64_t)table_bytes < abc_ancestor_table_bytes(N, d))
    return set_error(ABC_ERR_WORKSPACE, "ancestor_table: buffer too small");
  const AncTable v = anc_table_view(table, N, d);
  hipStream_t s = as_stream(stream);
  ABC_HIP(hipMemsetAsync(table, 0, ANC_HDR, s));
  hipLaunchKernelGGL(anc_records_kernel, dim3((unsigned)ceil_div(N * v.rs, 256)), dim3(256), 0,
                     s, X, cdf, N, d, v.rs, const_cast<double*>(v.rec));
  ABC_LAUNCHED();
  const int64_t nx = N * (int64_t)d;
  const int64_t xb = ceil_div(nx, 256) < XMAX_BLOCKS ? ceil_div(nx, 256) : XMAX_BLOCKS;
  hipLaunchKernelGGL(anc_xmax_kernel, dim3((unsigned)xb), dim3(256), 0, s, X, nx,
                     static_cast<unsigned long long*>(table));
  ABC_LAUNCHED();
  hipLaunchKernelGGL(anc_guide_kernel, dim3((unsigned)ceil_div(v.G + 2, 256)), dim3(256), 0, s,
                     cdf, N, v.G, const_cast<int32_t*>(v.guide));
  ABC_LAUNCHED();
  return ABC_OK;
}

extern "C" int abc_candidates_round(const abc_candidate_spec* spec, int64_t idx0,
                                    int64_t B, double eps, const double* eps_dev,
                                    double eps_scale, int filter, int64_t cap,
                                    int64_t* idx, int64_t* count, double* rec_x,
                                    void* ws, size_t ws_bytes, void* stream) {
  const int rc = check_spec(spec);
  if (rc != ABC_OK) return rc;
  ABC_CHECK_ARG(B >= 0 && cap >= 0 && count, "candidates_round: bad B/cap/count");
  ABC_CHECK_ARG(B < (1ll << 40), "candidates_round: B too large");
  ABC_CHECK_ARG(cap == 0 || idx, "candidates_round: null idx");
  RoundWs w;
  ABC_CARVE(w, "candidates_round", B);
  hipStream_t s = as_stream(stream);
  if (B == 0) {
    ABC_HIP(hipMemsetAsync(count, 0, sizeof(int64_t), s));
    return ABC_OK;
  }
  const double p = spec->p;
  const int filt = (filter && rec_x == nullptr && spec->S > 4 &&
                    (p == 1.0 || p == 2.0 || p == INFINITY)) ? 1 : 0;
  const int64_t nt = ceil_div(B, FR_TILE);
  ABC_CHECK_ARG(nt < (1ll << 31), "candidates_round: too many tiles");
  const double* box = spec->support_box;
  if (!box) {
    hipLaunchKernelGGL(support_box_kernel, dim3((unsigned)spec->d), dim3(64), 0, s,
                       spec->prior_kind, spec->prior_params, spec->d, w.box);
    ABC_LAUNCHED();
    box = w.box;
  }
  RoundArgs A = round_args(spec, box);
  A.eps_dev = eps_dev;
  A.eps_scale = eps_scale;
  profile_start(s, ABC_PROF_CANDIDATES);
  dispatch_spec(spec, [&](auto D, auto MODE) {
    launch_round<D(), MODE()>(filt != 0, p == 2.0, A, idx0, B, eps, w.bits, w.ticket, rec_x, s);
  });
  profile_stop(s, ABC_PROF_CANDIDATES);
  ABC_LAUNCHED();
  return compact_accept_bits(w.bits, w.rtot, B, cap, idx, count, s);
}

extern "C" int abc_pnorm_accept(const double* x, int64_t B, int S, const double* x0,
                                const double* wf, double p, double eps,
                                const int32_t* attempts, int max_attempts, int64_t cap,
                                int64_t* idx, int64_t* count, void* ws, size_t ws_bytes,
                                void* stream) {
  ABC_CHECK_ARG(S >= 1 && B >= 0 && p >= 1.0 && cap >= 0, "pnorm_accept: bad S/B/p/cap");
  ABC_CHECK_ARG(B < (1ll << 40), "pnorm_accept: B too large");
  ABC_CHECK_ARG(count && (cap == 0 || idx), "pnorm_accept: null pointer");
  RoundWs w;
  ABC_CARVE(w, "pnorm_accept", B);
  hipStream_t s = as_stream(stream);
  if (B == 0) {
    ABC_HIP(hipMemsetAsync(count, 0, sizeof(int64_t), s));
    return ABC_OK;
  }
  ABC_CHECK_ARG(x && x0 && wf, "pnorm_accept: null pointer");
  const int64_t nt = ceil_div(B, FR_TILE);
  ABC_CHECK_ARG(nt < (1ll << 31), "pnorm_accept: too many tiles");
  uint64_t* bits = w.bits;
  if (S <= 32)
    hipLaunchKernelGGL(pnorm_accept_kernel<false>, dim3((unsigned)nt), dim3(FR_T),
                       (size_t)pa_chunk_rows(S) * (S + 1) * sizeof(double), s, x, B, S, x0, wf, p, eps,
                       attempts, max_attempts, bits);
  else
    hipLaunchKernelGGL(pnorm_accept_kernel<true>, dim3((unsigned)nt), dim3(FR_T), 0, s, x, B,
                       S, x0, wf, p, eps, attempts, max_attempts, bits);
  ABC_LAUNCHED();
  return compact_accept_bits(bits, w.rtot, B, cap, idx, count, s);
}

extern "C" int abc_aggregate_accept(const double* x, int64_t B, int S, const double* x0,
                                    const double* wf, const double* p, const double* c, int K,
                                    double eps, const int32_t* attempts, int max_attempts,
                                    int64_t cap, int64_t* idx, int64_t* count, void* ws,
                                    size_t ws_bytes, void* stream) {
  AggTerms T;
  const int rc = agg_check_terms("aggregate_accept", S, p, c, K, T);
  if (rc != ABC_OK) return rc;
  ABC_CHECK_ARG(B >= 0 && cap >= 0, "aggregate_accept: bad B/cap");
  ABC_CHECK_ARG(B < (1ll << 40), "aggregate_accept: B too large");
  ABC_CHECK_ARG(count && (cap == 0 || idx), "aggregate_accept: null pointer");
  RoundWs w;
  ABC_CARVE(w, "aggregate_accept", B);
  hipStream_t s = as_stream(stream);
  if (B == 0) {
    ABC_HIP(hipMemsetAsync(count, 0, sizeof(int64_t), s));
    return ABC_OK;
  }
  ABC_CHECK_ARG(x && x0 && wf, "aggregate_accept: null pointer");
  const int64_t nt = ceil_div(B, S <= 32 ? AGG_TILE_ROW : AGG_TILE_WAVE);
  ABC_CHECK_ARG(nt < (1ll << 31), "aggregate_accept: too many tiles");
  auto launch = [&](auto kernel) {
    hipLaunchKernelGGL(kernel, dim3((unsigned)nt), dim3(FR_T), 0, s, x, B, S, x0, wf, T, eps,
                       attempts, max_attempts, w.bits);
  };
  if (S <= 32) launch(aggregate_accept_kernel<false, false>);
  else if (agg_simple(T.p, K)) launch(aggregate_accept_kernel<true, true>);
  else launch(aggregate_accept_kernel<true, false>);
  ABC_LAUNCHED();
  return compact_accept_bits(w.bits, w.rtot, B, cap, idx, count, s);
}

extern "C" int abc_prior_support_box(const int32_t* prior_kind, const double* prior_params,
                                     int d, double* box, void* stream) {
  ABC_CHECK_ARG(d >= 1 && d <= 64, "prior_support_box: bad d");
  ABC_CHECK_ARG(prior_kind && prior_params && box, "prior_support_box: null pointer");
  hipLaunchKernelGGL(support_box_kernel, dim3((unsigned)d), dim3(64), 0, as_stream(stream),
                     prior_kind, prior_params, d, box);
  ABC_LAUNCHED();
  return ABC_OK;
}

extern "C" int abc_round_keep(const int64_t* counts, int nranks, int rank, int64_t need,
                              int64_t* keep, void* stream) {
  ABC_CHECK_ARG(counts && keep && nranks >= 1 && rank >= 0 && rank < nranks,
                "round_keep: bad arguments");
  hipLaunchKernelGGL(round_keep_kernel, dim3(1), dim3(64), 0, as_stream(stream), counts, rank,
                     need, keep);
  ABC_LAUNCHED();
  return ABC_OK;
}

struct ProposeWs {
  double* box;
  void carve(Carver& c) { box = c.take<double>(128); }
};

extern "C" size_t abc_candidates_propose_workspace() { return measure<ProposeWs>(); }

extern "C" int abc_candidates_propose(const abc_candidate_spec* spec, int64_t idx0, int64_t B,
                                      double* theta, double* prior_logpdf, int64_t* ancestor,
                                      int32_t* attempts, void* ws, size_t ws_bytes,
                                      void* stream) {
  const int rc = check_spec(spec);
  if (rc != ABC_OK) return rc;
  ABC_CHECK_ARG(B >= 0 && B < (1ll << 40), "candidates_propose: bad B");
  if (B == 0) return ABC_OK;
  ABC_CHECK_ARG(theta, "candidates_propose: null pointer");
  ProposeWs w;
  ABC_CARVE(w, "candidates_propose");
  hipStream_t s = as_stream(stream);
  double* box = w.box;
  if (spec->support_box) {
    box = const_cast<double*>(spec->support_box);
  } else {
    hipLaunchKernelGGL(support_box_kernel, dim3((unsigned)spec->d), dim3(64), 0, s,
                       spec->prior_kind, spec->prior_params, spec->d, box);
    ABC_LAUNCHED();
  }
  const RoundArgs A = round_args(spec, box);
  const int64_t nb = ceil_div(B, (int64_t)FR_T * FP_CPT);
  ABC_CHECK_ARG(nb < (1ll << 31), "candidates_propose: too many blocks");
  dispatch_spec(spec, [&](auto D, auto MODE) {
    hipLaunchKernelGGL((fused_propose_kernel<D(), MODE()>), dim3((unsigned)nb), dim3(256), 0, s,
                       A, idx0, B, theta, prior_logpdf, ancestor, attempts);
  });
  ABC_LAUNCHED();
  return ABC_OK;
}

extern "C" int abc_candidates_regen(const abc_candidate_spec* spec, int64_t idx0,
                                    const int64_t* idx, int64_t n, const int64_t* n_dev,
                                    double* theta, double* prior_logpdf, int64_t* ancestor,
                                    double* x, double* dist, void* stream) {
  const int rc = check_spec(spec);
  if (rc != ABC_OK) return rc;
  ABC_CHECK_ARG(n >= 0, "candidates_regen: n < 0");
  if (n == 0) return ABC_OK;
  ABC_CHECK_ARG(idx && theta && prior_logpdf && x && dist, "candidates_regen: null pointer");
  const RoundArgs A = round_args(spec, nullptr);
  hipStream_t s = as_stream(stream);
  profile_start(s, ABC_PROF_REGEN);
  dispatch_spec(spec, [&](auto D, auto MODE) {
    hipLaunchKernelGGL((fused_regen_kernel<D(), MODE()>), dim3((unsigned)ceil_div(n, 256)),
                       dim3(256), 0, s, A, idx0, idx, n, n_dev, theta, prior_logpdf, ancestor, x,
                       dist);
  });
  profile_stop(s, ABC_PROF_REGEN);
  ABC_LAUNCHED();
  return ABC_OK;
}
```

### pyabc_amd/gpu.py

```python
import math

import numpy as np

from . import _native as nat

try:
    import torch
except ImportError:
    torch = None

F64 = None if torch is None else torch.float64
I64 = None if torch is None else torch.int64


class NoDeviceError(RuntimeError):
    pass


_have_device = False


def require_device():
    global _have_device
    if not _have_device:
        if torch is None or not torch.cuda.is_available():
            raise NoDeviceError("pyabc_amd GPU path needs an MI355X (HIP device)")
        nat.load()
        _have_device = True
    return torch.device("cuda", torch.cuda.current_device())


def stream_ptr():
    return torch._C._cuda_getCurrentRawStream(torch.cuda.current_device())


def p(t):
    if t is None:
        return None
    assert t.is_contiguous(), "kernels take contiguous tensors"
    return t.data_ptr()


_ws = {}


def workspace(nbytes, slot="main"):
    dev = torch.cuda.current_device()
    key = (dev, slot)
    buf = _ws.get(key)
    nbytes = max(int(nbytes), 256)
    if buf is None or buf.numel() < nbytes:
        buf = torch.zeros(int(nbytes * 1.25) + 256, dtype=torch.uint8,
                          device=f"cuda:{dev}")
        _ws[key] = buf
    return buf


class HostFuture:

    _events = {}

    def __init__(self, t, _record=True):
        self._h = torch.empty(t.shape, dtype=t.dtype, pin_memory=True)
        self._h.copy_(t, non_blocking=True)
        self._dev = t.device.index if t.is_cuda else torch.cuda.current_device()
        self._pooled = _record
        self._ev = None
        if _record:
            pool = HostFuture._events.setdefault(self._dev, [])
            self._ev = pool.pop() if pool else torch.cuda.Event()
            self._ev.record(torch.cuda.current_stream(self._dev))
        self._v = None

    @classmethod
    def group(cls, ts):
        futs = [cls(t, _record=False) for t in ts]
        if futs:
            ev = torch.cuda.Event()
            ev.record(torch.cuda.current_stream(futs[-1]._dev))
            for f in futs:
                f._ev = ev
        return futs

    def get(self):
        if self._v is None:
            self._ev.synchronize()
            self._v = self._h.numpy().copy()
            pool = HostFuture._events.setdefault(self._dev, [])
            if self._pooled and len(pool) < 64:
                pool.append(self._ev)
            self._h = self._ev = None
        return self._v

    def __deepcopy__(self, memo):
        return self

    def __getstate__(self):
        return {"_v": self.get(), "_h": None, "_ev": None}


_flat = {}


def flat_prior(d, device):
    key = (int(d), str(device))
    if key not in _flat:
        _flat[key] = (as_dev(np.full(d, -1), dtype=torch.int32, device=device),
                      torch.zeros(4 * d, dtype=F64, device=device))
    return _flat[key]


def as_dev(a, dtype=None, device=None):
    dtype = dtype or F64
    device = device or require_device()
    if isinstance(a, torch.Tensor):
        return a.to(device=device, dtype=dtype).contiguous()
    return torch.as_tensor(np.ascontiguousarray(a), dtype=dtype,
                           device=device).contiguous()



def weighted_moments(X, w, with_max=False):
    N, d = X.shape
    out = torch.empty(3 + d + d * d, dtype=F64, device=X.device)
    nb = nat.query("abc_weighted_moments_workspace", N, d)
    ws = workspace(nb)
    nat.call("abc_weighted_moments", p(X), p(w), N, d, p(out), p(ws), ws.numel(),
             stream_ptr())
    o = out.cpu().numpy()
    res = (o[0], o[1], o[2:2 + d].copy(), o[2 + d:2 + d + d * d].reshape(d, d).copy())
    return res + (o[2 + d + d * d],) if with_max else res


def inclusive_scan(x, out=None):
    n = x.numel()
    out = torch.empty_like(x) if out is None else out
    nb = nat.query("abc_scan_workspace", n)
    ws = workspace(nb, "scan")
    nat.call("abc_inclusive_scan_f64", p(x), p(out), n, p(ws), ws.numel(),
             stream_ptr())
    return out


def normalize_weights(w):
    n = w.numel()
    stats = torch.empty(3, dtype=F64, device=w.device)
    nb = nat.query("abc_normalize_weights_workspace", n)
    ws = workspace(nb, "norm")
    nat.call("abc_normalize_weights", p(w), n, p(stats), p(ws), ws.numel(),
             stream_ptr())
    return stats



def mvn_pack(X, w, mu, U, shift, prec, with_range=False, shift_dev=None):
    N, d = X.shape
    r = U.shape[1]
    nb = nat.query("abc_mvn_packed_bytes", N, r, prec)
    packed = torch.empty(nb, dtype=torch.uint8, device=X.device)
    rng = torch.empty(2, dtype=F64, device=X.device) if with_range else None
    nat.call("abc_mvn_pack_population", p(X), p(w), N, d, p(mu), p(U), r,
             float(shift), p(shift_dev), prec, p(packed), p(rng), stream_ptr())
    return (packed, rng) if with_range else packed


def weighted_moments_dev(X, w):
    N, d = X.shape
    out = torch.empty(3 + d + d * d, dtype=F64, device=X.device)
    nb = nat.query("abc_weighted_moments_workspace", N, d)
    ws = workspace(nb)
    nat.call("abc_weighted_moments", p(X), p(w), N, d, p(out), p(ws), ws.numel(),
             stream_ptr())
    return out


def mvn_fit(moments, d, scaling, bw_rule):
    dev = moments.device
    blob = torch.empty(4 * d * d + d + 8, dtype=F64, device=dev)
    cov, evec, U, L = (blob[k * d * d:(k + 1) * d * d].view(d, d) for k in range(4))
    evals = blob[4 * d * d:4 * d * d + d]
    stats = blob[4 * d * d + d:]
    nat.call("abc_mvn_fit", p(moments), d, float(scaling), int(bw_rule), p(cov), p(evec),
             p(evals), p(U), p(L), p(stats), stream_ptr())
    return cov, evec, evals, U, L, stats


def mvn_logpdf(x, packed, N, mu, U, prec, log_const, out=None, X=None, w=None,
               shift=0.0, hint=None):
    M, d = x.shape
    r = U.shape[1]
    out = torch.empty(M, dtype=F64, device=x.device) if out is None else out
    if M == 0:
        return out
    if hint is not None:
        if hint.dtype != I64 or hint.numel() != M:
            raise ValueError("mvn_logpdf: hint must be int64 [M]")
        hint = hint.contiguous()
    nb = nat.query("abc_mvn_logpdf_workspace", M, N, r, prec)
    ws = workspace(nb, "mvn")
    nat.call("abc_mvn_logpdf", p(x), M, d, p(packed), p(X), p(w), N, p(mu),
             p(U), r, prec, float(log_const), float(shift), p(out), p(hint),
             p(ws), ws.numel(), stream_ptr())
    return out


def mvn_x3_layout(r):
    import ctypes
    k, ct = ctypes.c_int(0), ctypes.c_int(0)
    kernel = int(nat.load().abc_mvn_x3_layout(int(r), ctypes.byref(k), ctypes.byref(ct)))
    return kernel, int(k.value), int(ct.value)


def mvn_x3_max_exponent():
    return int(nat.load().abc_mvn_x3_max_exponent())


def mvn_logpdf_direct(x, X, w, U, V, support_tol, log_const, out=None):
    M, d = x.shape
    N = X.shape[0]
    r = 0 if U is None else U.shape[1]
    nv = 0 if V is None else V.shape[1]
    out = torch.empty(M, dtype=F64, device=x.device) if out is None else out
    if M == 0:
        return out
    nat.call("abc_mvn_logpdf_direct", p(x), M, p(X), p(w), N, d,
             p(U) if r else None, r, p(V) if nv else None, nv,
             float(support_tol), float(log_const), p(out), stream_ptr())
    return out



def cdf_guide(cdf):
    N = cdf.numel()
    guide = torch.empty(N, dtype=torch.int32, device=cdf.device)
    nat.call("abc_cdf_guide", p(cdf), N, p(guide), stream_ptr())
    return guide


def ancestor_table(X, cdf):
    N, d = X.shape
    nb = nat.query("abc_ancestor_table_bytes", int(N), int(d))
    t = torch.empty(int(nb), dtype=torch.uint8, device=X.device)
    if t.data_ptr() % 128:
        raise RuntimeError("ancestor_table: allocation not 128-byte aligned")
    nat.call("abc_ancestor_table", p(X), p(cdf), int(N), int(d), p(t), t.numel(),
             stream_ptr())
    return t


def propose(X, cdf, L, prior_kind, prior_params, seed, generation, idx0, B,
            max_attempts, d, per_particle_L=False, guide=None):
    dev = prior_params.device
    theta = torch.empty((B, d), dtype=F64, device=dev)
    lp = torch.empty(B, dtype=F64, device=dev)
    anc = torch.empty(B, dtype=I64, device=dev)
    att = torch.empty(B, dtype=torch.int32, device=dev)
    N = 0 if X is None else X.shape[0]
    fn = "abc_local_propose" if per_particle_L else "abc_propose"
    nat.call(fn, p(X), p(cdf), p(guide), N, d, p(L), p(prior_kind), p(prior_params),
             int(seed) & (2 ** 64 - 1), int(generation) & 0xFFFFFFFF, int(idx0),
             int(B), int(max_attempts), p(theta), p(lp), p(anc), p(att),
             stream_ptr())
    return theta, lp, anc, att


def prior_logpdf(theta, prior_kind, prior_params, out=None):
    B, d = theta.shape
    out = torch.empty(B, dtype=F64, device=theta.device) if out is None else out
    nat.call("abc_prior_logpdf", p(theta), B, d, p(prior_kind), p(prior_params),
             p(out), stream_ptr())
    return out


def simulate_linear_gaussian(theta, src, a, sigma, seed, generation, idx0,
                             out=None):
    B, d = theta.shape
    S = src.numel()
    out = torch.empty((B, S), dtype=F64, device=theta.device) if out is None else out
    nat.call("abc_simulate_linear_gaussian", p(theta), B, d, S, p(src), p(a),
             p(sigma), int(seed) & (2 ** 64 - 1), int(generation) & 0xFFFFFFFF,
             int(idx0), p(out), stream_ptr())
    return out


def pnorm(x, x0, wf, pval, out=None):
    B, S = x.shape
    out = torch.empty(B, dtype=F64, device=x.device) if out is None else out
    nat.call("abc_pnorm", p(x), B, S, p(x0), p(wf), float(pval), p(out),
             stream_ptr())
    return out


def pnorm_accept(x, x0, wf, pval, eps, cap, att=None, max_attempts=0):
    B, S = x.shape
    if x.dtype != F64 or not x.is_contiguous():
        x = x.to(F64).contiguous()
    cap = int(min(max(cap, 0), B))
    idx = torch.empty(max(cap, 1), dtype=I64, device=x.device)
    cnt = torch.empty(1, dtype=I64, device=x.device)
    nb = nat.query("abc_candidates_workspace", int(B))
    ws = workspace(nb, "candidates")
    nat.call("abc_pnorm_accept", p(x), int(B), int(S), p(x0), p(wf), float(pval),
             float(eps), p(att), int(max_attempts), cap, p(idx), p(cnt), p(ws),
             ws.numel(), stream_ptr())
    return idx, cnt


class TermStack:

    def __init__(self, wf, pvals, c):
        pvals = np.ascontiguousarray(pvals, dtype=np.float64)
        c = np.ascontiguousarray(c, dtype=np.float64)
        K = int(pvals.size)
        if wf.dim() != 2 or wf.shape[0] != K or c.size != K:
            raise ValueError("TermStack: wf [K, S], p [K] and c [K] disagree")
        self.wf, self.K = wf, K
        self.p_host, self.c_host = pvals, c

    def args(self):
        return (p(self.wf), self.p_host.ctypes.data, self.c_host.ctypes.data, self.K)


def aggregate_distance(x, x0, stack, out=None, terms=False):
    B, S = x.shape
    if x.dtype != F64 or not x.is_contiguous():
        x = x.to(F64).contiguous()
    if stack.wf.shape[1] != S:
        raise ValueError(f"aggregate_distance: weights for {stack.wf.shape[1]} "
                         f"statistics, rows of {S}")
    out = torch.empty(B, dtype=F64, device=x.device) if out is None else out
    tm = torch.empty((B, stack.K), dtype=F64, device=x.device) if terms else None
    if B == 0:
        return (out, tm) if terms else out
    nat.call("abc_aggregate_distance", p(x), int(B), int(S), p(x0), *stack.args(),
             p(out), p(tm), stream_ptr())
    return (out, tm) if terms else out


def aggregate_accept(x, x0, stack, eps, cap, att=None, max_attempts=0):
    B, S = x.shape
    if x.dtype != F64 or not x.is_contiguous():
        x = x.to(F64).contiguous()
    if stack.wf.shape[1] != S:
        raise ValueError(f"aggregate_accept: weights for {stack.wf.shape[1]} "
                         f"statistics, rows of {S}")
    cap = int(min(max(cap, 0), B))
    idx = torch.empty(max(cap, 1), dtype=I64, device=x.device)
    cnt = torch.empty(1, dtype=I64, device=x.device)
    nb = nat.query("abc_candidates_workspace", int(B))
    ws = workspace(nb, "candidates")
    nat.call("abc_aggregate_accept", p(x), int(B), int(S), p(x0), *stack.args(),
             float(eps), p(att), int(max_attempts), cap, p(idx), p(cnt), p(ws),
             ws.numel(), stream_ptr())
    return idx, cnt


class PNormTail:

    def __init__(self, wf, pval):
        self.wf, self.pval = wf, pval

    def accept(self, x, x0, eps, cap, att=None, max_attempts=0):
        return pnorm_accept(x, x0, self.wf, self.pval, eps, cap, att=att,
                            max_attempts=max_attempts)

    def distances(self, rows, x0):
        return pnorm(rows, x0, self.wf, self.pval)


class AggregateTail:

    def __init__(self, stack):
        self.stack = stack

    def accept(self, x, x0, eps, cap, att=None, max_attempts=0):
        return aggregate_accept(x, x0, self.stack, eps, cap, att=att,
                                max_attempts=max_attempts)

    def distances(self, rows, x0):
        return aggregate_distance(rows, x0, self.stack)


def prior_uniforms(att, k, seed, generation, idx0, B=None):
    B = att.numel() if B is None else B
    dev = att.device if att is not None else require_device()
    u = torch.empty(B, dtype=F64, device=dev)
    nat.call("abc_prior_uniforms", p(att) if att is not None else None, p(u), B, int(k),
             int(seed) & 0xFFFFFFFFFFFFFFFF, int(generation) & 0xFFFFFFFF, int(idx0),
             stream_ptr())
    return u


def mask_gave_up(dist, att, max_attempts, value=float("nan")):
    nat.call("abc_mask_gave_up", p(dist), p(att), dist.numel(), int(max_attempts),
             float(value), stream_ptr())
    return dist


def accept_compact(d, eps, idx_out=None, count_out=None):
    B = d.numel()
    idx = torch.empty(max(B, 1), dtype=I64, device=d.device) if idx_out is None else idx_out
    cnt = torch.empty(1, dtype=I64, device=d.device) if count_out is None else count_out
    nb = nat.query("abc_compact_workspace", B)
    ws = workspace(nb, "compact")
    nat.call("abc_accept_compact", p(d), B, float(eps), p(idx), p(cnt), p(ws),
             ws.numel(), stream_ptr())
    return idx, cnt


class CandidateRound:

    def __init__(self, d, S, prior_kind, prior_params, src, a, sigma, x0, wf,
                 p, seed, generation, max_attempts, X=None, cdf=None,
                 guide=None, L=None, per_particle_L=False, anc_table=None):
        self._keep = [t for t in (prior_kind, prior_params, src, a, sigma, x0,
                                  wf, X, cdf, guide, L, anc_table) if t is not None]
        for t in self._keep:
            assert t.is_contiguous() and t.is_cuda
        if src.dtype != torch.int32 or prior_kind.dtype != torch.int32:
            raise TypeError("CandidateRound: src / prior_kind must be int32")
        self.d, self.S = int(d), int(S)
        self.spec = nat.CandidateSpec()
        s = self.spec
        s.d, s.S = self.d, self.S
        s.X, s.cdf, s.guide = _ptr(X), _ptr(cdf), _ptr(guide)
        s.N = 0 if X is None else int(X.shape[0])
        s.L, s.per_particle_L = _ptr(L), int(bool(per_particle_L))
        s.prior_kind, s.prior_params = _ptr(prior_kind), _ptr(prior_params)
        s.max_attempts = int(max_attempts)
        s.src, s.a, s.sigma = _ptr(src), _ptr(a), _ptr(sigma)
        s.x0, s.wf, s.p = _ptr(x0), _ptr(wf), float(p)
        s.seed = int(seed) & (2 ** 64 - 1)
        s.generation = int(generation) & 0xFFFFFFFF
        if X is not None and anc_table is None:
            anc_table = ancestor_table(X, cdf)
            self._keep.append(anc_table)
        s.anc_table = _ptr(anc_table) if X is not None else None
        self._box = torch.empty(2 * self.d, dtype=F64, device=prior_params.device)
        nat.call("abc_prior_support_box", _ptr(prior_kind), _ptr(prior_params), self.d,
                 _ptr(self._box), stream_ptr())
        s.support_box = _ptr(self._box)
        self.device = prior_params.device

    def run(self, idx0, B, eps, cap, filter=True, rec_x=None, idx_out=None,
            count_out=None, eps_dev=None, eps_scale=1.0):
        import ctypes as C
        idx = (torch.empty(max(int(cap), 1), dtype=I64, device=self.device)
               if idx_out is None else idx_out)
        cnt = (torch.empty(1, dtype=I64, device=self.device)
               if count_out is None else count_out)
        if rec_x is not None and tuple(rec_x.shape) != (int(B), self.S):
            raise ValueError("CandidateRound.run: rec_x must be [B, S]")
        nb = nat.query("abc_candidates_workspace", int(B))
        ws = workspace(nb, "candidates")
        nat.call("abc_candidates_round", C.addressof(self.spec), int(idx0), int(B),
                 float(eps), p(eps_dev), float(eps_scale), int(bool(filter)), int(cap),
                 p(idx), p(cnt), p(rec_x),
                 p(ws), ws.numel(), stream_ptr())
        return idx, cnt

    def propose(self, idx0, B, with_lp=True):
        import ctypes as C
        dev = self.device
        B = int(B)
        theta = torch.empty((B, self.d), dtype=F64, device=dev)
        lp = torch.empty(B, dtype=F64, device=dev) if with_lp else None
        anc = torch.empty(B, dtype=I64, device=dev)
        att = torch.empty(B, dtype=torch.int32, device=dev)
        if B:
            ws = workspace(nat.query("abc_candidates_propose_workspace"), "propose")
            nat.call("abc_candidates_propose", C.addressof(self.spec), int(idx0), B,
                     p(theta), p(lp), p(anc), p(att), p(ws), ws.numel(), stream_ptr())
        return theta, lp, anc, att

    def regen(self, idx0, idx, out=None):
        import ctypes as C
        n = int(idx.numel())
        dev = self.device
        if out is not None:
            theta, lp, anc, x, dist = out
            if not (tuple(theta.shape) == (n, self.d) and lp.numel() == n and anc.numel() == n
                    and tuple(x.shape) == (n, self.S) and dist.numel() == n
                    and anc.dtype == I64 and all(t.is_contiguous() for t in out)):
                raise ValueError("CandidateRound.regen: out does not match the rows")
        else:
            theta = torch.empty((n, self.d), dtype=F64, device=dev)
            lp = torch.empty(n, dtype=F64, device=dev)
            anc = torch.empty(n, dtype=I64, device=dev)
            x = torch.empty((n, self.S), dtype=F64, device=dev)
            dist = torch.empty(n, dtype=F64, device=dev)
        if n:
            nat.call("abc_candidates_regen", C.addressof(self.spec), int(idx0),
                     p(idx.contiguous()), n, None, p(theta), p(lp), p(anc), p(x), p(dist),
                     stream_ptr())
        return theta, lp, anc, x, dist

    def regen_into(self, idx0, idx_ptr, n, ptrs, n_dev=None):
        import ctypes as C
        if n:
            nat.call("abc_candidates_regen", C.addressof(self.spec), int(idx0), idx_ptr,
                     int(n), p(n_dev), *ptrs, stream_ptr())


def round_keep(counts, need, rank, out=None):
    out = torch.empty(1, dtype=I64, device=counts.device) if out is None else out
    nat.call("abc_round_keep", p(counts), int(counts.numel()), int(rank), int(need), p(out),
             stream_ptr())
    return out


def _ptr(t):
    return None if t is None else p(t)


def gather_rows(x, idx, n=None):
    n = idx.numel() if n is None else n
    cols = 1 if x.dim() == 1 else x.shape[1]
    out = torch.empty((n, cols) if x.dim() > 1 else (n,), dtype=F64,
                      device=x.device)
    nat.call("abc_gather_rows", p(x), p(idx), n, cols, p(out), stream_ptr())
    return out


def gather_rows_batch(arrays, idx, n=None):
    import ctypes as C
    n = idx.numel() if n is None else int(n)
    outs = [torch.empty((n,) + tuple(a.shape[1:]), dtype=a.dtype, device=a.device)
            for a in arrays]
    if n == 0:
        return outs
    k = len(arrays)
    ins_c = (C.c_void_p * k)(*[p(a) for a in arrays])
    outs_c = (C.c_void_p * k)(*[p(o) for o in outs])
    cols_c = (C.c_int * k)(*[1 if a.dim() == 1 else int(a.shape[1]) for a in arrays])
    row0_c = (C.c_int64 * k)(*([0] * k))
    nat.call("abc_gather_rows_batch", k, C.addressof(ins_c), C.addressof(cols_c),
             C.addressof(outs_c), C.addressof(row0_c), p(idx), n, stream_ptr())
    return outs


def importance_weights(prior_lp, trans_lp, scale=1.0, acc_w=None):
    A = prior_lp.numel()
    w = torch.empty(A, dtype=F64, device=prior_lp.device)
    nat.call("abc_importance_weights", p(prior_lp), p(trans_lp), p(acc_w), A,
             float(scale), p(w), stream_ptr())
    return w



def sort_pairs(keys, vals):
    N = keys.numel()
    ko = torch.empty_like(keys)
    vo = torch.empty_like(vals)
    nb = nat.query("abc_sort_pairs_workspace", N)
    ws = workspace(nb, "sort")
    nat.call("abc_sort_pairs_f64", p(keys), p(vals), N, p(ko), p(vo), p(ws),
             ws.numel(), stream_ptr())
    return ko, vo


def weighted_quantile(points, w, alpha, sorted_path=False):
    N = points.numel()
    q = torch.empty(1, dtype=F64, device=points.device)
    name = "abc_weighted_quantile_sorted" if sorted_path else "abc_weighted_quantile"
    nb = nat.query(name + "_workspace", N)
    ws = workspace(nb, "sort" if sorted_path else "quantile")
    nat.call(name, p(points), p(w), N, float(alpha), p(q), p(ws), ws.numel(), stream_ptr())
    return q


def resolve_quantile(q_host, points, w, alpha):
    v = float(q_host)
    if v != v:
        v = float(weighted_quantile(points, w, alpha, sorted_path=True).cpu()[0])
    return v


def column_std(X):
    R, S = X.shape
    out = torch.empty(S, dtype=F64, device=X.device)
    nb = nat.query("abc_column_stats_workspace", R, S)
    ws = workspace(nb, "colstats")
    nat.call("abc_column_std", p(X), R, S, p(out), p(ws), ws.numel(), stream_ptr())
    return out


def column_mad(X):
    R, S = X.shape
    out = torch.empty(S, dtype=F64, device=X.device)
    nb = nat.query("abc_column_stats_workspace", R, S)
    ws = workspace(nb, "colstats")
    nat.call("abc_column_mad", p(X), R, S, p(out), p(ws), ws.numel(), stream_ptr())
    return out


def column_scale(X, kind, x0=None):
    R, S = X.shape
    kind = nat.SCALE_KINDS[kind] if isinstance(kind, str) else int(kind)
    if x0 is not None and x0.numel() != S:
        raise ValueError(f"column_scale: {x0.numel()} observations for {S} columns")
    out = torch.empty(S, dtype=F64, device=X.device)
    nb = nat.query("abc_column_scale_workspace", kind, R, S)
    ws = workspace(nb, "colstats")
    nat.call("abc_column_scale", kind, p(X), R, S, p(x0), p(out), p(ws),
             ws.numel(), stream_ptr())
    return out


def column_span(V):
    R, K = V.shape
    out = torch.empty(K, dtype=F64, device=V.device)
    nb = nat.query("abc_column_stats_workspace", R, K)
    ws = workspace(nb, "colstats")
    nat.call("abc_column_span", p(V), R, K, p(out), p(ws), ws.numel(), stream_ptr())
    return out


def bootstrap_cv(logdens, w, scale=1.0):
    B, N = logdens.shape
    if w.numel() != N or not logdens.is_contiguous():
        raise ValueError(f"bootstrap_cv: {w.numel()} weights for {N} test "
                         "points (or non-contiguous densities)")
    var = torch.empty(N, dtype=F64, device=logdens.device)
    cv = torch.empty(1, dtype=F64, device=logdens.device)
    nb = nat.query("abc_bootstrap_cv_workspace", N)
    ws = workspace(nb, "cv")
    nat.call("abc_bootstrap_cv", p(logdens), B, N, p(w), float(scale), p(var),
             p(cv), p(ws), ws.numel(), stream_ptr())
    return var, cv



def local_fit(X, w, k, scaling, eps):
    N, d = X.shape
    dev = X.device
    covs = torch.empty((N, d, d), dtype=F64, device=dev)
    inv = torch.empty_like(covs)
    chol = torch.empty_like(covs)
    dets = torch.empty(N, dtype=F64, device=dev)
    lnorm = torch.empty(N, dtype=F64, device=dev)
    nb = nat.query("abc_local_fit_workspace", N, d)
    ws = workspace(nb, "local")
    nat.call("abc_local_fit", p(X), p(w), N, d, int(k), float(scaling),
             float(eps), p(covs), p(inv), p(dets), p(chol), p(lnorm), p(ws),
             ws.numel(), stream_ptr())
    return covs, inv, dets, chol, lnorm


FIT_ROUTE_NAMES = ((nat.ABC_FIT_KNN, "knn"), (nat.ABC_FIT_LIST, "list"),
                   (nat.ABC_FIT_DENSE, "dense"), (nat.ABC_FIT_DEFER, "defer"),
                   (nat.ABC_FIT_DENSE_REJECTED, "rejected"),
                   (nat.ABC_FIT_SELECT_FALLBACK, "select-fallback"))


def local_fit_route():
    return int(nat.load().abc_local_fit_route())


def local_fit_route_names(route=None):
    route = local_fit_route() if route is None else route
    return "+".join(n for f, n in FIT_ROUTE_NAMES if route & f) or "plain"


def local_logpdf(x, X, w, inv, lnorm, out=None):
    M, d = x.shape
    N = X.shape[0]
    out = torch.empty(M, dtype=F64, device=x.device) if out is None else out
    if M == 0:
        return out
    ws = workspace(nat.query("abc_local_logpdf_workspace", M, N, d), "local_pdf")
    nat.call("abc_local_logpdf", p(x), M, p(X), p(w), N, d, p(inv), p(lnorm),
             p(out), p(ws), ws.numel(), stream_ptr())
    return out


def local_logpdf_route(M, N, d):
    import ctypes
    ws = workspace(nat.query("abc_local_logpdf_workspace", M, N, d), "local_pdf")
    direct, bound = ctypes.c_int64(0), ctypes.c_double(0.0)
    nat.call("abc_local_logpdf_route", M, N, d, p(ws), ws.numel(), stream_ptr(),
             ctypes.addressof(direct), ctypes.addressof(bound))
    return int(direct.value), bound.value


LOG_2PI = math.log(2 * math.pi)



KERNEL_KINDS = {"independent_normal": 0, "independent_laplace": 1,
                "normal": 2, "poisson": 3, "binomial": 4,
                "negative_binomial": 5}


def kernel_logpdf(x, cols, x0k, kind, par, c, U=None, ret_lin=False,
                  out=None):
    B, S = x.shape
    K = int(cols.numel())
    r = 0 if U is None else int(U.shape[1])
    out = torch.empty(B, dtype=F64, device=x.device) if out is None else out
    nat.call("abc_kernel_logpdf", p(x), B, S, p(cols), K, p(x0k),
             KERNEL_KINDS[kind], p(par), p(U), r, float(c), int(bool(ret_lin)),
             p(out), stream_ptr())
    return out


def stochastic_accept(dens, pdf_norm, temperature, scale_log, apply_iw, seed,
                      generation, idx0):
    B = dens.numel()
    key = torch.empty(B, dtype=F64, device=dens.device)
    accw = torch.empty(B, dtype=F64, device=dens.device)
    nat.call("abc_stochastic_accept", p(dens), B, float(pdf_norm),
             float(temperature), int(bool(scale_log)), int(bool(apply_iw)),
             int(seed) & (2 ** 64 - 1), int(generation) & 0xFFFFFFFF,
             int(idx0), p(key), p(accw), stream_ptr())
    return key, accw


TEMPER_ACCEPTANCE, TEMPER_ESS, TEMPER_MAX, TEMPER_ACCEPTANCE_LIN = 0, 1, 2, 3


def temper_sums(dens, lr, pdf_norm, scale_log, mode, beta=0.0, shift=0.0,
                lr_sub=None):
    R = lr.numel()
    if lr_sub is not None and lr_sub.numel() != R:
        raise ValueError("temper_sums: lr / lr_sub sizes differ")
    out = torch.empty(2, dtype=F64, device=lr.device)
    ws = workspace(nat.query("abc_temper_workspace"), "temper")
    nat.call("abc_temper_sums", p(dens), p(lr), p(lr_sub), R, float(pdf_norm),
             int(bool(scale_log)), int(mode), float(beta), float(shift),
             p(out), p(ws), ws.numel(), stream_ptr())
    a, b = out.cpu().numpy()
    return float(a), float(b)
```

Baseline: 7.522 million.

## Add coarse run table to ancestor guide for single-ancestor bin resolution

Builds an extra run table over groups of guide bins: when a whole group of 32 bins maps to a single ancestor, the draw resolves directly without reading the per-bin guide bracket or searching. A host registry reads back counters from the build through pinned memory and an event, then chooses per table whether to launch the new RUNS kernel variants for the filter and plain paths, using share thresholds. The aim is to save guide loads and search work in ancestor selection. In exchange it adds a table-build kernel, a possible host synchronisation when the mode is decided, and duplicate kernel instantiations.

```diff
diff --git a/include/abcgpu.h b/include/abcgpu.h
--- a/include/abcgpu.h
+++ b/include/abcgpu.h
@@ -135,6 +135,12 @@
 int64_t abc_ancestor_table_bytes(int64_t N, int d);
 int abc_ancestor_table(const double* X, const double* cdf, int64_t N, int d,
                        void* table, size_t table_bytes, void* stream);
+#define ABC_RUN_AUTO 0
+#define ABC_RUN_OFF 1
+#define ABC_RUN_ON 2
+int abc_ancestor_table_ex(const double* X, const double* cdf, int64_t N, int d,
+                          void* table, size_t table_bytes, int run_mode, void* stream);
+int abc_ancestor_table_stats(const void* table, int64_t* out);
 size_t abc_candidates_workspace(int64_t B);
 int abc_candidates_round(const abc_candidate_spec* spec, int64_t idx0,
                          int64_t B, double eps, const double* eps_dev,
diff --git a/pyabc_amd/_native.py b/pyabc_amd/_native.py
--- a/pyabc_amd/_native.py
+++ b/pyabc_amd/_native.py
@@ -39,6 +39,8 @@
     "abc_cdf_guide": (I32, [P, I64, P, P]),
     "abc_ancestor_table_bytes": (I64, [I64, I32]),
     "abc_ancestor_table": (I32, [P, P, I64, I32, P, SZ, P]),
+    "abc_ancestor_table_ex": (I32, [P, P, I64, I32, P, SZ, I32, P]),
+    "abc_ancestor_table_stats": (I32, [P, P]),
     "abc_propose": (I32, [P, P, P, I64, I32, P, P, P, U64, U32, I64, I64, I32,
                           P, P, P, P, P]),
     "abc_prior_logpdf": (I32, [P, I64, I32, P, P, P, P]),
@@ -127,6 +129,8 @@
 ABC_PROF_DENSITY, ABC_PROF_CANDIDATES, ABC_PROF_REGEN, ABC_PROF_RESCUE = 0, 1, 2, 3
 (ABC_FIT_KNN, ABC_FIT_LIST, ABC_FIT_DENSE, ABC_FIT_DEFER, ABC_FIT_DENSE_REJECTED,
  ABC_FIT_SELECT_FALLBACK) = 1, 2, 4, 8, 16, 32
+ABC_RUN_AUTO, ABC_RUN_OFF, ABC_RUN_ON = 0, 1, 2
+RUN_MODES = {"auto": ABC_RUN_AUTO, "off": ABC_RUN_OFF, "on": ABC_RUN_ON}
 ABC_PREC_F64 = 0
 ABC_PREC_F32 = 1
 ABC_PREC_X3 = 2
diff --git a/pyabc_amd/csrc/abc_candidate.h b/pyabc_amd/csrc/abc_candidate.h
--- a/pyabc_amd/csrc/abc_candidate.h
+++ b/pyabc_amd/csrc/abc_candidate.h
@@ -347,6 +347,12 @@
 };
 
 constexpr int ANC_HDR = 256;
+constexpr int ANC_HDR_RESOLVED = 1, ANC_HDR_RUNS = 2, ANC_HDR_SHIFT = 3, ANC_HDR_SERIAL = 4;
+constexpr int ANC_RUN_SHIFT = 5;
+__host__ __device__ inline const int32_t* anc_run_table(const int32_t* bguide, int64_t G) {
+  return bguide + (G + 2);
+}
+__host__ __device__ inline int64_t anc_runs(int64_t G) { return (G >> ANC_RUN_SHIFT) + 1; }
 __host__ __device__ inline int anc_rs(int d) { return (d + 1 + 15) / 16 * 16; }
 __host__ __device__ inline int64_t anc_bins(int64_t N) {
   const int64_t g = 4 * N;
@@ -424,7 +430,7 @@
   __syncthreads();
 }
 
-template <int D, int MODE, bool TABLE = false>
+template <int D, int MODE, bool TABLE = false, bool RUNS = false>
 __device__ __forceinline__ int propose_one(const ProposalArgs& A, const BlockConsts& C,
                                            uint64_t g, double* th, int64_t& j) {
   constexpr bool LT_LDS = MODE == PROP_MVN && D > 0 && D <= LT_DMAX;
@@ -447,16 +453,25 @@
       u32x4 r = ra;
       const double target = uniform53(ra.x, ra.y) * total;
       AncestorBracket br;
-      if (TABLE) {
+      int32_t kt32 = 0, rj = -1;
+      if (TABLE && RUNS) {
+        kt32 = (int32_t)anc_bin(target, C.inv_step, A.G);
+        rj = anc_run_table(A.bguide, A.G)[kt32 >> ANC_RUN_SHIFT];
+      } else if (TABLE) {
         const int64_t kt = anc_bin(target, C.inv_step, A.G);
         br = {A.bguide[kt], A.bguide[kt + 1]};
       } else {
         br = ancestor_bracket(A.guide, A.N, total, target);
       }
+      auto run_bracket = [&]() {
+        if (rj >= 0) br = {rj, rj};
+        else br = {A.bguide[kt32], A.bguide[kt32 + 1]};
+      };
 #pragma unroll
       for (int k = 0; k < (D > 0 ? D : d); ++k) th[k] = 0.0;
       const double* Lj = A.L;
       if (MODE == PROP_LOCAL) {
+        if (TABLE && RUNS) run_bracket();
         j = TABLE ? table_finish(A.rec, A.rs, d, A.N, target, br)
                   : ancestor_finish(A.cdf, A.N, target, br);
         Lj = A.L + j * d * d;
@@ -481,9 +496,11 @@
       };
 #pragma unroll 1
       for (int q = 0; q < d; q += 2) pair(q);
-      if (MODE != PROP_LOCAL)
+      if (MODE != PROP_LOCAL) {
+        if (TABLE && RUNS) run_bracket();
         j = TABLE ? table_finish(A.rec, A.rs, d, A.N, target, br)
                   : ancestor_finish(A.cdf, A.N, target, br);
+      }
       const double* Xj = TABLE ? A.rec + j * A.rs : A.X + j * d;
 #pragma unroll
       for (int k = 0; k < (D > 0 ? D : d); ++k) th[k] = Xj[k] + th[k];
@@ -646,7 +663,7 @@
   }
 }
 
-template <int D, int PK, int CG>
+template <int D, int PK, int CG, bool RUNS = false>
 __device__ __forceinline__ void lazy_head_group(const ProposalArgs& A, const SimDistArgs& M,
                                                 const BlockConsts& C, const uint64_t (&g)[CG],
                                                 double eps, bool (&keep)[CG]) {
@@ -666,15 +683,37 @@
     az[c] = r.z;
     aw[c] = r.w;
     const int64_t kt = anc_bin(target[c], C.inv_step, A.G);
-    glo[c] = A.bguide[kt];
-    ghi[c] = A.bguide[kt + 1];
+    if (RUNS) {
+      glo[c] = anc_run_table(A.bguide, A.G)[kt >> ANC_RUN_SHIFT];
+      ghi[c] = (int32_t)kt;
+    } else {
+      glo[c] = A.bguide[kt];
+      ghi[c] = A.bguide[kt + 1];
+    }
+  }
+  u32x4 rp[CG];
+  if constexpr (RUNS) {
+#pragma unroll
+    for (int c = 0; c < CG; ++c) rp[c] = philox(g[c], SLOT_PERTURB, A.gen, A.seed);
+#pragma unroll
+    for (int c = 0; c < CG; ++c) {
+      const int32_t rj = glo[c], kt = ghi[c];
+      if (rj < 0) {
+        glo[c] = A.bguide[kt];
+        ghi[c] = A.bguide[kt + 1];
+      } else {
+        ghi[c] = rj;
+      }
+    }
   }
   double th[CG][KT];
 #pragma unroll
   for (int c = 0; c < CG; ++c) {
 #pragma unroll
     for (int k = 0; k < KT; ++k) th[c][k] = 0.0;
-    const u32x4 r = philox(g[c], SLOT_PERTURB, A.gen, A.seed);
+    u32x4 r;
+    if constexpr (RUNS) r = rp[c];
+    else r = philox(g[c], SLOT_PERTURB, A.gen, A.seed);
 #pragma unroll
     for (int q = 0; q < KT; q += 2) {
       double n0, n1;
diff --git a/pyabc_amd/csrc/abc_fused.hip b/pyabc_amd/csrc/abc_fused.hip
--- a/pyabc_amd/csrc/abc_fused.hip
+++ b/pyabc_amd/csrc/abc_fused.hip
@@ -1,5 +1,6 @@
 #include "abc_candidate.h"
 #include "abc_aggregate.h"
+#include <mutex>
 
 namespace abc {
 namespace {
@@ -18,11 +19,11 @@
   double eps_scale;
 };
 
-template <int D, int MODE, int PK>
+template <int D, int MODE, int PK, bool RUNS = false>
 __device__ __forceinline__ double evaluate_full(const RoundArgs& A, const BlockConsts& C,
                                                 uint64_t g,
                                                 double* th, int64_t& j, int& att, double* x) {
-  att = propose_one<D, MODE, true>(A.P, C, g, th, j);
+  att = propose_one<D, MODE, true, RUNS>(A.P, C, g, th, j);
   const double s = sim_pnorm<D, PK>(A.M, C, th, g, A.P.gen, A.P.seed, 0, A.M.S, 0.0, x);
   const double dist = pnorm_finish<PK>(s, A.M.p);
   return att <= A.P.max_attempts ? dist : NAN;
@@ -68,7 +69,7 @@
   uint16_t* queue;
   int& qn;
 };
-template <int D, int MODE, bool FILTER, int PK>
+template <int D, int MODE, bool FILTER, int PK, bool RUNS = false>
 __device__ __forceinline__ void tile_body(const RoundArgs& A, const BlockConsts& C, double eps,
                                           int64_t idx0, int64_t B, int64_t tile0, int cpt,
                                           uint64_t* __restrict__ bits,
@@ -92,7 +93,7 @@
           bool keep[FR_CG];
 #pragma unroll
           for (int c = 0; c < FR_CG; ++c) gs[c] = (uint64_t)(idx0 + tile0 + (it + c) * FR_T + tid);
-          lazy_head_group<D, PK, FR_CG>(A.P, A.M, C, gs, eps, keep);
+          lazy_head_group<D, PK, FR_CG, RUNS>(A.P, A.M, C, gs, eps, keep);
 #pragma unroll
           for (int c = 0; c < FR_CG; ++c) {
             const int loc = (it + c) * FR_T + tid;
@@ -111,7 +112,7 @@
       const int64_t b = tile0 + loc;
       if (b < B) {
         const uint64_t g = (uint64_t)(idx0 + b);
-        att = propose_one<D, MODE, true>(A.P, C, g, th, j);
+        att = propose_one<D, MODE, true, RUNS>(A.P, C, g, th, j);
         const double s = sim_pnorm<D, PK>(A.M, C, th, g, A.P.gen, A.P.seed, 0, 4, 0.0, nullptr);
         if (att <= A.P.max_attempts && !(pnorm_finish<PK>(s, A.M.p) > eps)) {
           const int pos = atomicAdd(&T.qn, 1);
@@ -128,8 +129,8 @@
     const int64_t b = tile0 + loc;
     if (b < B) {
       double* xr = rec_x ? rec_x + b * A.M.S : nullptr;
-      const double dist = evaluate_full<D, MODE, PK>(A, C, (uint64_t)(idx0 + b), th, j, att,
-                                                  xr);
+      const double dist = evaluate_full<D, MODE, PK, RUNS>(A, C, (uint64_t)(idx0 + b), th, j,
+                                                        att, xr);
       if (dist <= eps) atomicOr(&T.tbits[loc >> 5], 1u << (loc & 31));
     }
   }
@@ -149,7 +150,7 @@
   else { tile0 = nbig * FR_TILE + (t - nbig) * FR_TILE_TAIL; cpt = FR_CPT_TAIL; }
 }
 
-template <int D, int MODE, bool FILTER, int PK>
+template <int D, int MODE, bool FILTER, int PK, bool RUNS = false>
 __device__ __forceinline__ void round_body(RoundArgs A, int64_t idx0, int64_t B,
                                            double eps_host, uint64_t* __restrict__ bits,
                                            unsigned int* __restrict__ ticket,
@@ -176,12 +177,12 @@
     int64_t tile0;
     int cpt;
     tile_span(t, nbig, tile0, cpt);
-    tile_body<D, MODE, FILTER, PK>(A, C, eps, idx0, B, tile0, cpt, bits, rec_x, T);
+    tile_body<D, MODE, FILTER, PK, RUNS>(A, C, eps, idx0, B, tile0, cpt, bits, rec_x, T);
     __syncthreads();
   }
 }
 
-template <int D, int MODE, int PK>
+template <int D, int MODE, int PK, bool RUNS = false>
 __device__ __forceinline__ void round_plain_body(RoundArgs A, int64_t idx0, int64_t B,
                                                  double eps_host, uint64_t* __restrict__ bits,
                                                  unsigned int* __restrict__ ticket,
@@ -226,7 +227,8 @@
       int64_t j;
       int att;
       double* xr = rec_x ? rec_x + b * A.M.S : nullptr;
-      const double dist = evaluate_full<D, MODE, PK>(A, C, (uint64_t)(idx0 + b), th, j, att, xr);
+      const double dist =
+          evaluate_full<D, MODE, PK, RUNS>(A, C, (uint64_t)(idx0 + b), th, j, att, xr);
       if (dist <= eps) atomicOr(&tbits[loc >> 5], 1u << (loc & 31));
     }
     ++it;
@@ -237,7 +239,7 @@
   return (!filter && PK == 2 && D == 10 && MODE != PROP_PRIOR) ? 6 : 1;
 }
 
-#define ABC_ROUND_KERNEL(NAME, FILTER, PK)                                                \
+#define ABC_ROUND_KERNEL(NAME, FILTER, PK, RUNS)                                          \
   template <int D, int MODE>                                                              \
   __global__ __launch_bounds__(FR_T, fr_min_waves(FILTER, D, MODE, PK))                   \
   void NAME(RoundArgs A, int64_t idx0, int64_t B,                                         \
@@ -245,14 +247,20 @@
                                                unsigned int* ticket, int64_t nbig,        \
                                                int64_t ntiles, double* rec_x) {           \
     if (FILTER)                                                                           \
-      round_body<D, MODE, true, PK>(A, idx0, B, eps, bits, ticket, nbig, ntiles, nullptr);\
+      round_body<D, MODE, true, PK, RUNS>(A, idx0, B, eps, bits, ticket, nbig, ntiles,    \
+                                          nullptr);                                       \
     else                                                                                  \
-      round_plain_body<D, MODE, PK>(A, idx0, B, eps, bits, ticket, nbig, ntiles, rec_x);  \
-  }
-ABC_ROUND_KERNEL(fused_round_plain, false, 0)
-ABC_ROUND_KERNEL(fused_round_plain_p2, false, 2)
-ABC_ROUND_KERNEL(fused_round_filter, true, 0)
-ABC_ROUND_KERNEL(fused_round_filter_p2, true, 2)
+      round_plain_body<D, MODE, PK, RUNS>(A, idx0, B, eps, bits, ticket, nbig, ntiles,    \
+                                          rec_x);                                         \
+  }
+ABC_ROUND_KERNEL(fused_round_plain, false, 0, false)
+ABC_ROUND_KERNEL(fused_round_plain_p2, false, 2, false)
+ABC_ROUND_KERNEL(fused_round_filter, true, 0, false)
+ABC_ROUND_KERNEL(fused_round_filter_p2, true, 2, false)
+ABC_ROUND_KERNEL(fused_round_plain_runs, false, 0, true)
+ABC_ROUND_KERNEL(fused_round_plain_p2_runs, false, 2, true)
+ABC_ROUND_KERNEL(fused_round_filter_runs, true, 0, true)
+ABC_ROUND_KERNEL(fused_round_filter_p2_runs, true, 2, true)
 #undef ABC_ROUND_KERNEL
 
 constexpr int RG_MAX = 2048;
@@ -353,10 +361,16 @@
 }
 
 template <int D, int MODE>
-void launch_round(bool filt, bool p2, const RoundArgs& A, int64_t idx0, int64_t B, double eps,
-                  uint64_t* bits, unsigned int* ticket, double* rec_x, hipStream_t s) {
+void launch_round(bool filt, bool p2, bool runs, const RoundArgs& A, int64_t idx0, int64_t B,
+                  double eps, uint64_t* bits, unsigned int* ticket, double* rec_x,
+                  hipStream_t s) {
   auto k = filt ? (p2 ? fused_round_filter_p2<D, MODE> : fused_round_filter<D, MODE>)
                 : (p2 ? fused_round_plain_p2<D, MODE> : fused_round_plain<D, MODE>);
+  if constexpr (MODE != PROP_PRIOR) {
+    if (runs)
+      k = filt ? (p2 ? fused_round_filter_p2_runs<D, MODE> : fused_round_filter_runs<D, MODE>)
+               : (p2 ? fused_round_plain_p2_runs<D, MODE> : fused_round_plain_runs<D, MODE>);
+  }
   const TilePlan p = plan_tiles(B, resident_blocks(k, FR_T));
   hipLaunchKernelGGL(k, dim3(p.grid), dim3(FR_T), 0, s, A, idx0, B, eps, bits, ticket, p.nbig,
                      p.ntiles, rec_x);
@@ -405,29 +419,36 @@
 }
 
 constexpr int FP_CPT = 4;
-template <int D, int MODE>
-__global__ __launch_bounds__(256) void fused_propose_kernel(
-    RoundArgs A, int64_t idx0, int64_t B, double* __restrict__ theta,
-    double* __restrict__ lp, int64_t* __restrict__ anc, int32_t* __restrict__ att_out) {
-  constexpr int DM = D > 0 ? D : 64;
-  __shared__ BlockConsts C;
-  stage_block_consts<D, MODE, true>(C, A.P, nullptr, A.box);
-  const int d = D > 0 ? D : A.P.d;
-  for (int c = 0; c < FP_CPT; ++c) {
-    const int64_t i = ((int64_t)blockIdx.x * FP_CPT + c) * FR_T + threadIdx.x;
-    if (i >= B) break;
-    double th[DM];
-    int64_t j = -1;
-    const int att = propose_one<D, MODE, true>(A.P, C, (uint64_t)(idx0 + i), th, j);
-    double* row = theta + i * d;
-#pragma unroll
-    for (int k = 0; k < DM; ++k)
-      if (k < d) row[k] = th[k];
-    if (lp) lp[i] = att <= A.P.max_attempts ? prior_logpdf(A.P.kind, A.P.params, d, th) : -INFINITY;
-    if (anc) anc[i] = j;
-    if (att_out) att_out[i] = att;
-  }
-}
+#define ABC_PROPOSE_KERNEL(NAME, RUNS)                                                      \
+  template <int D, int MODE>                                                                \
+  __global__ __launch_bounds__(256) void NAME(                                              \
+      RoundArgs A, int64_t idx0, int64_t B, double* __restrict__ theta,                     \
+      double* __restrict__ lp, int64_t* __restrict__ anc, int32_t* __restrict__ att_out) {  \
+    constexpr int DM = D > 0 ? D : 64;                                                      \
+    __shared__ BlockConsts C;                                                               \
+    stage_block_consts<D, MODE, true>(C, A.P, nullptr, A.box);                              \
+    const int d = D > 0 ? D : A.P.d;                                                        \
+                    \
+    for (int c = 0; c < FP_CPT; ++c) {                                                      \
+      const int64_t i = ((int64_t)blockIdx.x * FP_CPT + c) * FR_T + threadIdx.x;            \
+      if (i >= B) break;                                                                    \
+      double th[DM];                                                                        \
+      int64_t j = -1;                                                                       \
+      const int att = propose_one<D, MODE, true, RUNS>(A.P, C, (uint64_t)(idx0 + i), th, j);\
+      double* row = theta + i * d;                                                          \
+      _Pragma("unroll")                                                                     \
+      for (int k = 0; k < DM; ++k)                                                          \
+        if (k < d) row[k] = th[k];                                                          \
+      if (lp)                                                                               \
+        lp[i] = att <= A.P.max_attempts ? prior_logpdf(A.P.kind, A.P.params, d, th)         \
+                                        : -INFINITY;                                        \
+      if (anc) anc[i] = j;                                                                  \
+      if (att_out) att_out[i] = att;                                                        \
+    }                                                                                       \
+  }
+ABC_PROPOSE_KERNEL(fused_propose_kernel, false)
+ABC_PROPOSE_KERNEL(fused_propose_runs_kernel, true)
+#undef ABC_PROPOSE_KERNEL
 
 __host__ __device__ constexpr int pa_chunk_rows(int S) {
   return (65536 / ((S + 1) * 8)) >= FR_T ? FR_T : ((65536 / ((S + 1) * 8)) & ~1);
@@ -611,6 +632,37 @@
   guide[k] = (int32_t)lo;
 }
 
+__global__ __launch_bounds__(256) void anc_run_kernel(const int32_t* __restrict__ guide,
+                                                      int64_t G, int64_t Gc, int64_t serial,
+                                                      int32_t* __restrict__ run,
+                                                      unsigned long long* __restrict__ hdr) {
+  __shared__ int wc[4];
+  const int64_t c = (int64_t)blockIdx.x * 256 + threadIdx.x;
+  bool res = false;
+  if (c < Gc) {
+    const int64_t lo = c << ANC_RUN_SHIFT, hi = lo + (1ll << ANC_RUN_SHIFT);
+    int32_t r = -1;
+    if (hi <= G + 1) {
+      const int32_t a = guide[lo];
+      if (a == guide[hi]) r = a;
+    }
+    run[c] = r;
+    res = r >= 0;
+  }
+  const int n = __popcll(__ballot(res));
+  if ((threadIdx.x & 63) == 0) wc[threadIdx.x >> 6] = n;
+  __syncthreads();
+  if (threadIdx.x == 0) {
+    const int tot = wc[0] + wc[1] + wc[2] + wc[3];
+    if (tot) atomicAdd(hdr + ANC_HDR_RESOLVED, (unsigned long long)tot);
+    if (blockIdx.x == 0) {
+      hdr[ANC_HDR_RUNS] = (unsigned long long)Gc;
+      hdr[ANC_HDR_SHIFT] = (unsigned long long)ANC_RUN_SHIFT;
+      hdr[ANC_HDR_SERIAL] = (unsigned long long)serial;
+    }
+  }
+}
+
 struct AncTable { const double* rec; const int32_t* guide; int rs; int64_t G; const double* xmax; };
 inline AncTable anc_table_view(const void* t, int64_t N, int d) {
   AncTable v;
@@ -620,6 +672,73 @@
   v.rec = reinterpret_cast<const double*>(static_cast<const char*>(t) + ANC_HDR);
   v.guide = reinterpret_cast<const int32_t*>(v.rec + N * v.rs);
   return v;
+}
+
+constexpr double ANC_RUN_TAU_FILTER = 0.13;
+constexpr double ANC_RUN_TAU_PLAIN = 0.65;
+constexpr int ANC_MODE_FILTER = 1, ANC_MODE_PLAIN = 2;
+constexpr int ANC_REG = 64;
+struct AncReg {
+  const void* table = nullptr;
+  int64_t N = 0, serial = 0;
+  int d = 0, want = ABC_RUN_AUTO;
+  int decided = -1;
+  int64_t Gc = 0, resolved = -1;
+  hipEvent_t ev = nullptr;
+};
+struct AncRegistry {
+  std::mutex mu;
+  AncReg e[ANC_REG];
+  int64_t (*pin)[4] = nullptr;
+  int64_t serial = 0;
+  int next = 0;
+};
+inline AncRegistry& anc_registry() {
+  static AncRegistry r;
+  return r;
+}
+inline int anc_reg_find(AncRegistry& r, const void* table) {
+  for (int i = 0; i < ANC_REG; ++i)
+    if (r.e[i].table == table) return i;
+  return -1;
+}
+inline bool anc_reg_counters(AncRegistry& r, int i) {
+  AncReg& e = r.e[i];
+  if (e.resolved >= 0) return true;
+  if (hipEventQuery(e.ev) != hipSuccess && hipEventSynchronize(e.ev) != hipSuccess) {
+    (void)hipGetLastError();
+    return false;
+  }
+  const volatile int64_t* h = r.pin[i];
+  if (h[ANC_HDR_SERIAL - 1] != e.serial) return false;
+  e.resolved = h[ANC_HDR_RESOLVED - 1];
+  e.Gc = h[ANC_HDR_RUNS - 1];
+  return true;
+}
+inline int anc_reg_mode(AncRegistry& r, int i) {
+  AncReg& e = r.e[i];
+  if (e.decided >= 0) return e.decided;
+  if (e.want == ABC_RUN_OFF) {
+    e.decided = 0;
+  } else if (e.want == ABC_RUN_ON) {
+    e.decided = ANC_MODE_FILTER | ANC_MODE_PLAIN;
+  } else {
+    e.decided = 0;
+    if (anc_reg_counters(r, i) && e.Gc > 1) {
+      const double share = (double)e.resolved / (double)(e.Gc - 1);
+      if (share >= ANC_RUN_TAU_FILTER) e.decided |= ANC_MODE_FILTER;
+      if (share >= ANC_RUN_TAU_PLAIN) e.decided |= ANC_MODE_PLAIN;
+    }
+  }
+  return e.decided;
+}
+inline bool spec_draws_runs(const abc_candidate_spec* s, int which) {
+  if (!s->X || !s->anc_table) return false;
+  AncRegistry& r = anc_registry();
+  std::lock_guard<std::mutex> lk(r.mu);
+  const int i = anc_reg_find(r, s->anc_table);
+  if (i < 0 || r.e[i].N != s->N || r.e[i].d != s->d) return false;
+  return (anc_reg_mode(r, i) & which) != 0;
 }
 
 RoundArgs round_args(const abc_candidate_spec* s, const double* box) {
@@ -683,13 +802,21 @@
 extern "C" int64_t abc_ancestor_table_bytes(int64_t N, int d) {
   if (N < 1 || d < 1) return 0;
   return ANC_HDR + N * anc_rs(d) * (int64_t)sizeof(double) +
-         (anc_bins(N) + 2) * (int64_t)sizeof(int32_t);
+         (anc_bins(N) + 2 + anc_runs(anc_bins(N))) * (int64_t)sizeof(int32_t);
 }
 
 extern "C" int abc_ancestor_table(const double* X, const double* cdf, int64_t N, int d,
                                   void* table, size_t table_bytes, void* stream) {
+  return abc_ancestor_table_ex(X, cdf, N, d, table, table_bytes, ABC_RUN_AUTO, stream);
+}
+
+extern "C" int abc_ancestor_table_ex(const double* X, const double* cdf, int64_t N, int d,
+                                     void* table, size_t table_bytes, int run_mode,
+                                     void* stream) {
   ABC_CHECK_ARG(N >= 1 && N < (1ll << 31) && d >= 1 && d <= 64,
                 "ancestor_table: bad N/d");
+  ABC_CHECK_ARG(run_mode == ABC_RUN_AUTO || run_mode == ABC_RUN_OFF || run_mode == ABC_RUN_ON,
+                "ancestor_table: bad run_mode");
   ABC_CHECK_ARG(X && cdf && table, "ancestor_table: null pointer");
   ABC_CHECK_ARG(((uintptr_t)table & 127) == 0, "ancestor_table: table not 128-B aligned");
   if ((int64_t)table_bytes < abc_ancestor_table_bytes(N, d))
@@ -708,6 +835,52 @@
   hipLaunchKernelGGL(anc_guide_kernel, dim3((unsigned)ceil_div(v.G + 2, 256)), dim3(256), 0, s,
                      cdf, N, v.G, const_cast<int32_t*>(v.guide));
   ABC_LAUNCHED();
+  AncRegistry& r = anc_registry();
+  std::lock_guard<std::mutex> lk(r.mu);
+  if (r.pin == nullptr)
+    ABC_HIP(hipHostMalloc(reinterpret_cast<void**>(&r.pin), sizeof(int64_t[4]) * ANC_REG,
+                          hipHostMallocDefault));
+  int i = anc_reg_find(r, table);
+  if (i < 0) {
+    i = r.next;
+    r.next = (r.next + 1) % ANC_REG;
+  }
+  AncReg& e = r.e[i];
+  if (e.ev) {
+    ABC_HIP(hipEventSynchronize(e.ev));
+  } else {
+    ABC_HIP(hipEventCreateWithFlags(&e.ev, hipEventDisableTiming));
+  }
+  e.table = table;
+  e.N = N;
+  e.d = d;
+  e.want = run_mode;
+  e.decided = -1;
+  e.resolved = -1;
+  e.Gc = 0;
+  e.serial = ++r.serial;
+  const int64_t Gc = anc_runs(v.G);
+  unsigned long long* hdr = static_cast<unsigned long long*>(table);
+  hipLaunchKernelGGL(anc_run_kernel, dim3((unsigned)ceil_div(Gc, 256)), dim3(256), 0, s, v.guide,
+                     v.G, Gc, e.serial,
+                     const_cast<int32_t*>(anc_run_table(v.guide, v.G)), hdr);
+  ABC_LAUNCHED();
+  ABC_HIP(hipMemcpyAsync(r.pin[i], hdr + 1, sizeof(int64_t[4]), hipMemcpyDeviceToHost, s));
+  ABC_HIP(hipEventRecord(e.ev, s));
+  return ABC_OK;
+}
+
+extern "C" int abc_ancestor_table_stats(const void* table, int64_t* out) {
+  ABC_CHECK_ARG(table && out, "ancestor_table_stats: null pointer");
+  AncRegistry& r = anc_registry();
+  std::lock_guard<std::mutex> lk(r.mu);
+  const int i = anc_reg_find(r, table);
+  ABC_CHECK_ARG(i >= 0, "ancestor_table_stats: not a table abc_ancestor_table built");
+  if (!anc_reg_counters(r, i))
+    return set_error(ABC_ERR_HIP, "ancestor_table_stats: the build's counters did not arrive");
+  out[0] = r.e[i].Gc;
+  out[1] = r.e[i].resolved;
+  out[2] = anc_reg_mode(r, i);
   return ABC_OK;
 }
 
@@ -741,11 +914,16 @@
     box = w.box;
   }
   RoundArgs A = round_args(spec, box);
+  const bool runs_head = spec_draws_runs(spec, ANC_MODE_FILTER);
+  const bool runs_plain = spec_draws_runs(spec, ANC_MODE_PLAIN);
   A.eps_dev = eps_dev;
   A.eps_scale = eps_scale;
   profile_start(s, ABC_PROF_CANDIDATES);
   dispatch_spec(spec, [&](auto D, auto MODE) {
-    launch_round<D(), MODE()>(filt != 0, p == 2.0, A, idx0, B, eps, w.bits, w.ticket, rec_x, s);
+    constexpr bool HEAD = MODE() == PROP_MVN && D() > LAZY_KT && D() <= LT_DMAX;
+    const bool runs = (filt && HEAD) ? runs_head : runs_plain;
+    launch_round<D(), MODE()>(filt != 0, p == 2.0, runs, A, idx0, B, eps, w.bits, w.ticket,
+                              rec_x, s);
   });
   profile_stop(s, ABC_PROF_CANDIDATES);
   ABC_LAUNCHED();
@@ -864,9 +1042,14 @@
   const RoundArgs A = round_args(spec, box);
   const int64_t nb = ceil_div(B, (int64_t)FR_T * FP_CPT);
   ABC_CHECK_ARG(nb < (1ll << 31), "candidates_propose: too many blocks");
+  const bool runs = spec_draws_runs(spec, ANC_MODE_PLAIN);
   dispatch_spec(spec, [&](auto D, auto MODE) {
-    hipLaunchKernelGGL((fused_propose_kernel<D(), MODE()>), dim3((unsigned)nb), dim3(256), 0, s,
-                       A, idx0, B, theta, prior_logpdf, ancestor, attempts);
+    auto k = fused_propose_kernel<D(), MODE()>;
+    if constexpr (MODE() != PROP_PRIOR) {
+      if (runs) k = fused_propose_runs_kernel<D(), MODE()>;
+    }
+    hipLaunchKernelGGL(k, dim3((unsigned)nb), dim3(256), 0, s, A, idx0, B, theta, prior_logpdf,
+                       ancestor, attempts);
   });
   ABC_LAUNCHED();
   return ABC_OK;
diff --git a/pyabc_amd/gpu.py b/pyabc_amd/gpu.py
--- a/pyabc_amd/gpu.py
+++ b/pyabc_amd/gpu.py
@@ -237,15 +237,22 @@
     return guide
 
 
-def ancestor_table(X, cdf):
+def ancestor_table(X, cdf, run_mode="auto"):
     N, d = X.shape
     nb = nat.query("abc_ancestor_table_bytes", int(N), int(d))
     t = torch.empty(int(nb), dtype=torch.uint8, device=X.device)
     if t.data_ptr() % 128:
         raise RuntimeError("ancestor_table: allocation not 128-byte aligned")
-    nat.call("abc_ancestor_table", p(X), p(cdf), int(N), int(d), p(t), t.numel(),
-             stream_ptr())
+    nat.call("abc_ancestor_table_ex", p(X), p(cdf), int(N), int(d), p(t), t.numel(),
+             nat.RUN_MODES[run_mode], stream_ptr())
     return t
+
+
+def ancestor_table_stats(table):
+    import ctypes as C
+    out = (C.c_int64 * 3)()
+    nat.call("abc_ancestor_table_stats", p(table), C.addressof(out))
+    return int(out[0]), int(out[1]), int(out[2])
 
 
 def propose(X, cdf, L, prior_kind, prior_params, seed, generation, idx0, B,
```

New measurement: 7.284 million. -3.2%, worse.
